# IuvenisSapiens/Qwen3-TTS-Rust

Hardware: AMD Instinct MI355X
Metric: audio-seconds generated per second (aggregate over GPUs) = concurrent real-time streams; RTF and first-chunk latency from the single-utterance leg (higher is better)
Workload: dtype i8

## Files before the change

### include/q3tts.h

```cpp
#ifndef Q3TTS_H
#define Q3TTS_H
#include <stdint.h>
#include <stddef.h>
#ifdef __cplusplus
extern "C" {
#endif

#define Q3TTS_OK 0
#define Q3TTS_ERR -1

const char* q3tts_last_error(void);
int q3tts_version(void);
int q3tts_device_count(void);

typedef struct q3tts_sampler_config {
    float temperature;
    int32_t top_k;
    float top_p;
    int32_t has_seed;
    uint64_t seed;
} q3tts_sampler_config;
void q3tts_sampler_config_default(q3tts_sampler_config* c);

typedef struct q3tts_gen_options {
// ... 236 lines not shown
int32_t q3tts_tokenizer_vocab_size(q3tts_tokenizer* t);
int64_t q3tts_text_nfc(const char* utf8, char* out, int64_t cap);

typedef struct q3tts_onnx q3tts_onnx;
int q3tts_onnx_open(const char* path, q3tts_onnx** out);
void q3tts_onnx_close(q3tts_onnx* m);
int q3tts_onnx_counts(q3tts_onnx* m, int32_t* n_nodes, int32_t* n_initializers, int32_t* n_inputs, int32_t* n_outputs);
int64_t q3tts_onnx_summary(q3tts_onnx* m, char* buf, int64_t cap);
int q3tts_onnx_node(q3tts_onnx* m, int32_t i, const char** op_type, const char** name, int32_t* n_in, int32_t* n_out, int32_t* n_attr);
const char* q3tts_onnx_node_input(q3tts_onnx* m, int32_t i, int32_t j);
const char* q3tts_onnx_node_output(q3tts_onnx* m, int32_t i, int32_t j);
int32_t q3tts_onnx_node_attr_ints(q3tts_onnx* m, int32_t i, const char* attr, int64_t* out, int32_t cap);
int32_t q3tts_onnx_node_attr_float(q3tts_onnx* m, int32_t i, const char* attr, float* out);
int q3tts_onnx_initializer(q3tts_onnx* m, int32_t i, const char** name, int32_t* dtype, int64_t* dims8, int32_t* ndims, const void** data,
                           int64_t* nbytes);
const char* q3tts_onnx_op_kernel(const char* op_type);
int q3tts_onnx_decoder_contract(q3tts_onnx* m, char* buf, int64_t cap);

typedef struct q3tts_onnx_session q3tts_onnx_session;
int q3tts_onnx_session_open(const char* path, int32_t device, q3tts_onnx_session** out);
void q3tts_onnx_session_close(q3tts_onnx_session* s);
int32_t q3tts_onnx_session_unsupported(q3tts_onnx_session* s, char* buf, int64_t cap);
int q3tts_onnx_session_set_input(q3tts_onnx_session* s, const char* name, int32_t dtype, const void* data, const int64_t* shape, int32_t rank);
int q3tts_onnx_session_run(q3tts_onnx_session* s);
int q3tts_onnx_session_output_info(q3tts_onnx_session* s, const char* name, int32_t* dtype, int32_t* rank, int64_t* shape8);
int q3tts_onnx_session_output(q3tts_onnx_session* s, const char* name, void* dst, int64_t cap_bytes);
int64_t q3tts_onnx_session_launches(q3tts_onnx_session* s);
int q3tts_onnx_op_executable(const char* op_type);
typedef struct q3tts_onnx_decoder q3tts_onnx_decoder;
int q3tts_onnx_decoder_open(const char* path, int32_t device, q3tts_onnx_decoder** out);
void q3tts_onnx_decoder_close(q3tts_onnx_decoder* d);
int q3tts_onnx_decoder_reset(q3tts_onnx_decoder* d);
int q3tts_onnx_decoder_decode(q3tts_onnx_decoder* d, const int64_t* codes, int32_t n_frames, int32_t is_final, float* pcm, int64_t cap, int64_t* n_out);
int q3tts_onnx_decoder_fetch(q3tts_onnx_decoder* d, float* pcm, int64_t cap, int64_t* n_out);

int q3tts_op_gemv_q8(const void* w_q8_0 , int32_t n, int32_t k, const int8_t* xq,
                     const uint16_t* xd, int32_t ntok, float* y , int32_t lpr);
int q3tts_op_gemv_kq(const void* const* raws, const int32_t* types, const int32_t* rows, int32_t nparts, int32_t k, const int8_t* xq, const uint16_t* xd,
                     int32_t ntok, float* y, int32_t lpr);
int q3tts_op_gateup_kq(const void* gate_raw, const void* up_raw, int32_t type, int32_t ff, int32_t k, const int8_t* xq, const uint16_t* xd, int32_t ntok,
                       int8_t* aq, uint16_t* ad);
int q3tts_op_gateup_q8(const void* w_q8_0, int32_t ff, int32_t k, const int8_t* xq, const uint16_t* xd, int32_t ntok, int8_t* aq,
                       uint16_t* ad);
int q3tts_op_matmul_float(const void* w , int32_t type, int32_t n, int32_t k, int32_t row0, int32_t nrows,
                          const float* x , int32_t ntok, float* y );
int q3tts_op_rmsnorm_quant(const float* x, const float* g, int32_t d, int32_t ntok, float eps, int8_t* xq, uint16_t* xd,
                           float* xn);
int q3tts_op_swiglu_quant(const float* gu, int32_t ff, int32_t ntok, int8_t* aq, uint16_t* ad);
int q3tts_op_argmax(const float* logits, int32_t n, int32_t start, int32_t end, int32_t mask_idx, int32_t* out);
int q3tts_op_sample(const float* logits, int32_t n, float temperature, int32_t top_k, float top_p, uint64_t seed, int32_t mask_idx,
                    int32_t n_draws, int32_t* out);
int q3tts_op_sample_rows(int32_t kernel, const float* logits, int32_t B, int32_t n, const float* temperature, const int32_t* top_k,
                         const float* top_p, const float* penalty, const uint64_t* seed, const int32_t* hist, const int32_t* hist_len,
                         int32_t hist_cap, int32_t n_draws, int32_t* out);
int q3tts_op_project(const float* x, const float* w , const float* b, int32_t n_in, int32_t n_out, float* y);
int q3tts_op_logprob_rows(const float* logits, int32_t B, int32_t n, int32_t stride, const int32_t* chosen, int32_t extra_idx,
                          float* out_chosen, float* out_extra);
int q3tts_op_score_rows(const float* tlogits, int32_t t_stride, const float* plogits, const int32_t* codes, int32_t F, float* out);
int q3tts_op_score_inputs(const float* hidden_proj, const float* const* tabs, const int64_t* tab_rows, int32_t dP, const int32_t* codes,
                          int32_t F, float* out);
int q3tts_op_kv_fork(uint16_t* k_cache, uint16_t* v_cache, int32_t n_pages, int32_t n_layer, int32_t n_kv, const int32_t* page_table,
                     int32_t n_seq, int32_t max_pages, int32_t src_seq, const int32_t* dst_seqs, int32_t n_dst, int32_t n_positions);
int q3tts_op_feedback_rows(const q3tts_assets* a, const int32_t* codes, int32_t n, const int32_t* trail_ids, int32_t n_trail, float* rows);
enum { Q3TTS_GEMM_AUTO = 0, Q3TTS_GEMM_SKINNY4 = 1, Q3TTS_GEMM_SKINNY8 = 2, Q3TTS_GEMM_SKINNY16 = 3,
       Q3TTS_GEMM_F32_1 = 4, Q3TTS_GEMM_F32_2 = 5,
       Q3TTS_GEMM_H1 = 6, Q3TTS_GEMM_H1_EPL = 7, Q3TTS_GEMM_H2 = 8, Q3TTS_GEMM_H2_EPL = 9,
       Q3TTS_GEMM_H3 = 10, Q3TTS_GEMM_H3_EPL = 11 };
enum { Q3TTS_EPI_NONE = 0, Q3TTS_EPI_GELU = 1, Q3TTS_EPI_RES_SCALE = 2 , Q3TTS_EPI_RES = 3 ,
       Q3TTS_EPI_SNAKE = 4  };
typedef struct q3tts_codec_gemm_desc {
    int32_t M, N, cin, taps, dil;
    const float* A; int64_t a_rows; int32_t lda, a_segT, a_skip;
    int32_t a_split, o_split;
    const float* W; const float* bias;
    int32_t epi; const float* res; int64_t res_floats; int32_t ldr, r_segT; int64_t r_skip;
    const float* scale; const float* snake_ea; const float* snake_ib;
    float* out; int64_t out_floats, out_off; int32_t ldo, o_segT; int64_t o_skip;
    int64_t ws_floats;
    int32_t form, ksplit, reducer;
    int32_t form_ran, ksplit_ran, reducer_ran;
} q3tts_codec_gemm_desc;
int q3tts_op_codec_gemm(q3tts_codec_gemm_desc* d);
int q3tts_codec_gemm_plan(q3tts_codec_gemm_desc* d);

enum { Q3TTS_CK_RVQ_SUM = 0, Q3TTS_CK_RMSNORM_ROWS = 1, Q3TTS_CK_LAYERNORM_ROWS = 2, Q3TTS_CK_ROPE_APPEND = 3, Q3TTS_CK_WINDOW_ATTN = 4,
       Q3TTS_CK_SWIGLU_ROWS = 5, Q3TTS_CK_DWCONV7 = 6, Q3TTS_CK_SNAKE = 7, Q3TTS_CK_SNAKE_SPLIT = 8, Q3TTS_CK_CONV_OUT_WAVE = 9,
       Q3TTS_CK_CONV_OUT_WIN = 10, Q3TTS_CK_HIST_LOAD = 11, Q3TTS_CK_HIST_SAVE = 12, Q3TTS_CK_HIST_ZERO = 13 };
typedef struct q3tts_codec_kernel_desc {
    int32_t kernel;
    int32_t G, T, C, H;
    int32_t n_heads, head_dim, window; float rope_base, eps, bias;
    const int64_t* meta;
    const int64_t* codes; int32_t n_q, cb_size;
    int32_t n_streams, stream;
    const float* in[3]; int64_t in_floats[3];
    const float* p0; const float* p1; int64_t p0_floats, p1_floats;
    float* out[3]; int64_t out_floats[3];
} q3tts_codec_kernel_desc;
int q3tts_op_codec_kernel(q3tts_codec_kernel_desc* d);

enum { Q3TTS_ATTN_AUTO = 0, Q3TTS_ATTN_UNFUSED = 1 , Q3TTS_ATTN_FUSED = 2 ,
       Q3TTS_ATTN_SHORT1 = 3, Q3TTS_ATTN_SHORT2 = 4 , Q3TTS_ATTN_GGML = 5  };
typedef struct q3tts_attention_desc {
    int32_t n_head, n_kv, n_layer, layer, ntok;
    const float* qkv; int32_t qkv_stride;
    const float* q_norm; const float* k_norm;
    float eps, rope_base; int32_t n_ctx; int32_t mrope_sec[4];
    const int32_t* seq; const int32_t* slot; const int32_t* pos; int32_t uniform_pos;
    const int32_t* page_table; int32_t n_seq, max_pages;
    uint16_t* k_cache; uint16_t* v_cache; int32_t n_pages;
    int32_t fused, fused_max_tok, same_seq, short_attn_min, hpw1_max, float_mode, ggml_mode;
    int32_t form;
    float* att; int8_t* aq; uint16_t* ad;
    int32_t form_ran;
} q3tts_attention_desc;
int q3tts_op_attention(q3tts_attention_desc* d);
int q3tts_op_attention_keyed(q3tts_attention_desc* d, const uint64_t* keys, int32_t key_stride, int32_t qkv_rows);
int q3tts_attention_plan(q3tts_attention_desc* d);

enum { Q3TTS_LOP_GEMV = 0, Q3TTS_LOP_GATEUP = 1, Q3TTS_LOP_NORM = 2, Q3TTS_LOP_NORM_GEMV = 3, Q3TTS_LOP_NORM_ARGMAX = 4, Q3TTS_LOP_NORM_GATEUP = 5,
       Q3TTS_LOP_F_GEMV = 6, Q3TTS_LOP_F_GATEUP = 7 };
enum { Q3TTS_LIN_AUTO = 0, Q3TTS_LIN_GEMV_Q8 = 1, Q3TTS_LIN_GEMM_Q8_TOK = 2, Q3TTS_LIN_GEMM_Q8_MFMA = 3, Q3TTS_LIN_GEMM_Q8_TILE1 = 4,
       Q3TTS_LIN_GEMV_KQ = 5, Q3TTS_LIN_GEMM_KQ_MFMA = 6, Q3TTS_LIN_GU_Q8_TILE1 = 7, Q3TTS_LIN_GU_Q8_MFMA = 8, Q3TTS_LIN_GU_KQ_MFMA = 9,
       Q3TTS_LIN_GU_UNFUSED = 10, Q3TTS_LIN_NORM = 11, Q3TTS_LIN_NORM_WG = 12, Q3TTS_LIN_GEMV_NORM = 13, Q3TTS_LIN_GEMV_NORM_ARGMAX = 14,
       Q3TTS_LIN_GU_SWIGLU_NORM = 15, Q3TTS_LIN_F_GEMV = 16, Q3TTS_LIN_F_MFMA16 = 17, Q3TTS_LIN_F_MFMA = 18, Q3TTS_LIN_F_GU_MFMA16 = 19,
       Q3TTS_LIN_F_GU_UNFUSED = 20 };
typedef struct q3tts_linear_desc {
    int32_t op, form;
    int32_t nw; const void* raw[3]; int32_t type[3]; int32_t rows[3]; int32_t kq_layout;
    int32_t K, row0, nrows, nrows_valid, ntok, ff;
    int32_t lpr, mt, ztiles;
    int32_t fused;
    const int8_t* xq; const uint16_t* xd; int32_t a_rows;
    const float* x; int64_t x_floats; int32_t x_off, x_stride;
    const float* h_in; int64_t h_floats; int32_t h_stride;
    const uint64_t* idx_keys; const int32_t* idx; int32_t idx_stride;
    const float* parts; int64_t parts_floats; int32_t nparts, parts_stride; int64_t parts_slab;
    const float* g; float eps;
    float* h_out; float* xn_out;
    int8_t* xq_out; uint16_t* xd_out;
    uint64_t* keys; int64_t n_keys; int32_t key_stride; const int32_t* mask_per_tok; int32_t idx_add;
    float* out; int64_t out_floats, out_off; int32_t out_stride;
    int8_t* aq; uint16_t* ad;
    int32_t form_ran, lpr_ran, mt_ran, z_ran;
} q3tts_linear_desc;
int q3tts_op_linear(q3tts_linear_desc* d);
int q3tts_linear_plan(q3tts_linear_desc* d);
uint64_t q3tts_argmax_key(float v, int32_t idx);

enum { Q3TTS_SEL_SAMPLE = 0, Q3TTS_SEL_SAMPLE_PRED = 1, Q3TTS_SEL_ARGMAX = 2, Q3TTS_SEL_ARGMAX_KEYS = 3 };
#define Q3TTS_SELECT_SENTINEL 0xA5C3F00D5A3C0FF1ull
typedef struct q3tts_select_desc {
    int32_t kernel;
    int32_t B, n, stride, row_off;
    const float* logits;
    const float* temperature; const int32_t* top_k; const float* top_p;
    const int32_t* mask_idx;
    const uint64_t* seed;
    const uint32_t* draw0;
    int32_t n_draws;
    const float* penalty; const int32_t* hist; const int32_t* hist_len; int32_t hist_cap; const int32_t* cur_code;
    int32_t out_stride;
    int32_t start, end, add;
    int32_t* tokens;
    uint64_t* out_raw;
    uint32_t* draws_out;
// ... 8 lines not shown
```

### qwen3-tts-rust_amd/csrc/capi_ops.cpp

```cpp
#include "../../include/q3tts.h"
#include "transformer.h"
#include "host_logic.h"
#include "kdev.h"
#include "codec.h"

using namespace q3;
#define Q3_API_BEGIN try {
#define Q3_API_END(failval) } catch (const std::exception& ex) { set_last_error(ex.what()); return failval; } catch (...) { set_last_error("unknown error"); return failval; }
static void require_gpu() {
    int n = 0;
    if (hipGetDeviceCount(&n) != hipSuccess || n <= 0) throw Error("no HIP device available: the HIP path is the only compute path (no CPU fallback)");
}

static int attention_op_plan(const q3tts_attention_desc& d) {
    AttnPlanIn a;
    a.ntok = d.ntok; a.fused = d.fused != 0; a.fused_max_tok = d.fused_max_tok; a.same_seq = d.same_seq != 0; a.short_attn_min = d.short_attn_min;
    a.n_head = d.n_head; a.n_kv = d.n_kv; a.hpw1_max = d.hpw1_max > 0 ? d.hpw1_max : short_attn_hpw1_max();
    a.float_mode = d.float_mode != 0; a.ggml_mode = d.ggml_mode != 0;
    return plan_attention(a);
}

static void attention_op_check(const q3tts_attention_desc& d, int form) {
    Q3_CHECK(form >= ATTN_UNFUSED && form <= ATTN_GGML, "unknown attention form");
    Q3_CHECK(d.n_head >= 1 && d.n_kv >= 1 && d.n_head % d.n_kv == 0, "n_head must be a multiple of n_kv");
// ... 718 lines not shown
        Q3_CHECK(d.hist && d.hist_len && d.hist_cap >= 1, "a penalty needs a history");
        for (int b = 0; b < B; b++) Q3_CHECK(d.hist_len[b] >= 0 && d.hist_len[b] <= d.hist_cap, "hist_len out of range");
    }
    const float guard = 3e38f;
    std::vector<float> hl((size_t)d.row_off + (size_t)B * d.stride, guard);
    for (int b = 0; b < B; b++) std::copy(d.logits + (size_t)b * n, d.logits + (size_t)(b + 1) * n, hl.begin() + d.row_off + (size_t)b * d.stride);
    DevBuf<float> dl(hl.size()); dl.upload(hl.data(), hl.size());
    const float* rows = dl.p + d.row_off;
    DevBuf<int32_t> dm;
    if (d.mask_idx) { dm.alloc(B); dm.upload(d.mask_idx, B); }
    const size_t slots = (size_t)B * d.out_stride;
    std::vector<q3_u64> raw((size_t)nl * slots);
    if (d.kernel == Q3TTS_SEL_ARGMAX) {
        const int32_t s32 = (int32_t)(uint32_t)(Q3TTS_SELECT_SENTINEL & 0xFFFFFFFFull);
        std::vector<int32_t> ho(slots, s32);
        DevBuf<int32_t> dout(slots); dout.upload(ho.data(), slots);
        launch_argmax(0, rows, d.stride, d.start, d.end, dm.p, dout.p, d.out_stride, d.add, B);
        Q3_LAUNCH_CHECK();
        Q3_HIP(hipDeviceSynchronize());
        dout.download(ho.data(), slots);
        for (size_t i = 0; i < slots; i++) raw[i] = (q3_u64)(uint32_t)ho[i];
        std::copy(raw.begin(), raw.end(), (q3_u64*)d.out_raw);
        for (int b = 0; b < B; b++) d.tokens[b] = ho[(size_t)b * d.out_stride];
        return Q3TTS_OK;
    }
    std::fill(raw.begin(), raw.end(), (q3_u64)Q3TTS_SELECT_SENTINEL);
    DevBuf<q3_u64> dout(raw.size()); dout.upload(raw.data(), raw.size());
    if (d.kernel == Q3TTS_SEL_ARGMAX_KEYS) {
        launch_argmax_keys(0, rows, d.stride, n, dm.p, dout.p, d.out_stride, B);
        Q3_LAUNCH_CHECK();
        Q3_HIP(hipDeviceSynchronize());
        dout.download((q3_u64*)d.out_raw, raw.size());
        for (int b = 0; b < B; b++) d.tokens[b] = key_code(d.out_raw[(size_t)b * d.out_stride]);
        return Q3TTS_OK;
    }
    DevBuf<float> dt(B), dp_(B), dpen; DevBuf<int32_t> dk(B), dh, dlen; DevBuf<uint32_t> dkey((size_t)8 * B), ddraw(B); DevBuf<q3_u64> dcur;
    dt.upload(d.temperature, B); dp_.upload(d.top_p, B); dk.upload(d.top_k, B);
    std::vector<uint32_t> keys((size_t)8 * B), draw(B, 0u);
    for (int b = 0; b < B; b++) { StdRng rng(d.seed[b]); std::copy(rng.key(), rng.key() + 8, keys.begin() + (size_t)b * 8); if (d.draw0) draw[b] = d.draw0[b]; }
    dkey.upload(keys.data(), keys.size()); ddraw.upload(draw.data(), B);
    SampleArgs a{rows, d.stride, n, dt.p, dk.p, dp_.p, dm.p, dkey.p, ddraw.p, dout.p, d.out_stride};
    if (d.penalty) {
        const size_t hs = (size_t)d.hist_cap * 16;
        std::vector<int32_t> hh((size_t)B * hs, 0);
        for (int b = 0; b < B; b++) for (int f = 0; f < d.hist_cap; f++) hh[(size_t)b * hs + (size_t)f * 16] = d.hist[(size_t)b * d.hist_cap + f];
        dh.alloc(hh.size()); dh.upload(hh.data(), hh.size()); dlen.alloc(B); dlen.upload(d.hist_len, B); dpen.alloc(B); dpen.upload(d.penalty, B);
        a.penalty = dpen.p; a.hist = dh.p; a.hist_stride = (int)hs; a.hist_len = dlen.p;
        if (d.cur_code) {
            std::vector<q3_u64> cur((size_t)16 * B, pack_key(0.0f, 0));
            for (int b = 0; b < B; b++) cur[(size_t)b * 16] = pack_key(0.0f, d.cur_code[b]);
            dcur.alloc(cur.size()); dcur.upload(cur.data(), cur.size());
            a.cur_key = dcur.p; a.cur_stride = 16;
        }
    }
    for (int i = 0; i < nl; i++) {
        a.out_key = dout.p + (size_t)i * slots;
        if (d.kernel == Q3TTS_SEL_SAMPLE) launch_sample(0, a, B);
        else launch_sample_pred(0, a, B);
        Q3_LAUNCH_CHECK();
    }
    Q3_HIP(hipDeviceSynchronize());
    dout.download((q3_u64*)d.out_raw, raw.size());
    ddraw.download(d.draws_out, B);
    for (int i = 0; i < nl; i++) for (int b = 0; b < B; b++) d.tokens[(size_t)i * B + b] = key_code(d.out_raw[(size_t)i * slots + (size_t)b * d.out_stride]);
    return Q3TTS_OK;
    Q3_API_END(Q3TTS_ERR)
}

int q3tts_op_codec_gemm(q3tts_codec_gemm_desc* d) {
    Q3_API_BEGIN
    require_gpu();
    codec_gemm_run(d);
    return Q3TTS_OK;
    Q3_API_END(Q3TTS_ERR)
}

int q3tts_codec_gemm_plan(q3tts_codec_gemm_desc* d) {
    Q3_API_BEGIN
    codec_gemm_plan_only(d);
    return Q3TTS_OK;
    Q3_API_END(Q3TTS_ERR)
}

int q3tts_op_codec_kernel(q3tts_codec_kernel_desc* d) {
    Q3_API_BEGIN
    require_gpu();
    codec_kernel_run(d);
    return Q3TTS_OK;
    Q3_API_END(Q3TTS_ERR)
}

int q3tts_op_project(const float* x, const float* w, const float* b, int32_t n_in, int32_t n_out, float* y) {
    Q3_API_BEGIN
    require_gpu();
    std::vector<float> wt((size_t)n_in * n_out);
    for (int o = 0; o < n_out; o++) for (int i = 0; i < n_in; i++) wt[(size_t)i * n_out + o] = w[(size_t)o * n_in + i];
    DevBuf<float> dx(n_in), dw(wt.size()), db(n_out), dy(n_out);
    dx.upload(x, n_in); dw.upload(wt.data(), wt.size()); db.upload(b, n_out);
    launch_project(0, dx.p, n_in, dw.p, db.p, n_in, n_out, dy.p, n_out, 1);
    Q3_HIP(hipDeviceSynchronize());
    dy.download(y, n_out);
    return Q3TTS_OK;
    Q3_API_END(Q3TTS_ERR)
}

int q3tts_mel_frames(int32_t n) { const int plen = n + 768; return (plen > 1024 ? plen - 1024 : 0) / 256 + 1; }

}

#include "onnx_reader.h"
#include "onnx_exec.h"
struct q3tts_onnx { std::unique_ptr<OnnxModel> m; std::string text; };
extern "C" {
int q3tts_onnx_open(const char* path, q3tts_onnx** out) {
    Q3_API_BEGIN
    Q3_CHECK(path && out, "null argument");
    auto* h = new q3tts_onnx();
    try { h->m.reset(new OnnxModel(path)); } catch (...) { delete h; throw; }
    *out = h;
    return Q3TTS_OK;
    Q3_API_END(Q3TTS_ERR)
}
void q3tts_onnx_close(q3tts_onnx* m) { delete m; }
int q3tts_onnx_counts(q3tts_onnx* m, int32_t* n_nodes, int32_t* n_init, int32_t* n_in, int32_t* n_out) {
    if (!m) return Q3TTS_ERR;
    if (n_nodes) *n_nodes = (int32_t)m->m->nodes.size();
    if (n_init) *n_init = (int32_t)m->m->initializers.size();
    if (n_in) *n_in = (int32_t)m->m->inputs.size();
    if (n_out) *n_out = (int32_t)m->m->outputs.size();
    return Q3TTS_OK;
}
int64_t q3tts_onnx_summary(q3tts_onnx* m, char* buf, int64_t cap) {
    if (!m) return -1;
    m->text = m->m->summary();
    if (buf && cap > 0) { const size_t n = std::min((size_t)cap - 1, m->text.size()); std::memcpy(buf, m->text.data(), n); buf[n] = 0; }
    return (int64_t)m->text.size() + 1;
}
int q3tts_onnx_node(q3tts_onnx* m, int32_t i, const char** op_type, const char** name, int32_t* n_in, int32_t* n_out, int32_t* n_attr) {
    Q3_API_BEGIN
    Q3_CHECK(m && i >= 0 && i < (int)m->m->nodes.size(), "node index out of range");
    const OnnxNode& n = m->m->nodes[i];
    if (op_type) *op_type = n.op_type.c_str();
    if (name) *name = n.name.c_str();
    if (n_in) *n_in = (int32_t)n.inputs.size();
    if (n_out) *n_out = (int32_t)n.outputs.size();
    if (n_attr) *n_attr = (int32_t)n.attrs.size();
    return Q3TTS_OK;
    Q3_API_END(Q3TTS_ERR)
}
const char* q3tts_onnx_node_input(q3tts_onnx* m, int32_t i, int32_t j) {
    return (m && i >= 0 && i < (int)m->m->nodes.size() && j >= 0 && j < (int)m->m->nodes[i].inputs.size()) ? m->m->nodes[i].inputs[j].c_str() : nullptr;
}
const char* q3tts_onnx_node_output(q3tts_onnx* m, int32_t i, int32_t j) {
    return (m && i >= 0 && i < (int)m->m->nodes.size() && j >= 0 && j < (int)m->m->nodes[i].outputs.size()) ? m->m->nodes[i].outputs[j].c_str() : nullptr;
}
int32_t q3tts_onnx_node_attr_ints(q3tts_onnx* m, int32_t i, const char* attr, int64_t* out, int32_t cap) {
    if (!m || i < 0 || i >= (int)m->m->nodes.size() || !attr) return -1;
    const OnnxAttr* a = m->m->nodes[i].attr(attr);
    if (!a) return -1;
    if (a->type == 2 || (a->ints.empty() && a->type == 0)) { if (out && cap > 0) out[0] = a->i; return 1; }
    for (int k = 0; k < (int)a->ints.size() && k < cap; k++) out[k] = a->ints[k];
    return (int32_t)a->ints.size();
}
int32_t q3tts_onnx_node_attr_float(q3tts_onnx* m, int32_t i, const char* attr, float* out) {
    if (!m || i < 0 || i >= (int)m->m->nodes.size() || !attr || !out) return -1;
    const OnnxAttr* a = m->m->nodes[i].attr(attr);
// ... 164 lines not shown
```

### qwen3-tts-rust_amd/csrc/codec.h

```cpp
#pragma once
#include "q3_common.h"
#include <memory>
#include <string>
#include <vector>

struct q3tts_codec_gemm_desc;
struct q3tts_codec_kernel_desc;

namespace q3 {

struct CodecStateEntry { std::string name; int64_t offset; int rows, cols; };

class CodecDecoder {
public:
    std::vector<CodecStateEntry> state_layout() const;
    size_t state_floats() const;
    void state_export(int stream, float* out, size_t n_floats) const;
    void state_import(int stream, const float* in, size_t n_floats);
    CodecDecoder(const std::string& gguf_path, int n_streams, int max_frames_per_call, int n_lanes = 1, int max_group = 1);
    int max_group() const;
    int n_lanes() const;
    ~CodecDecoder();
    int samples_per_frame() const;
    void reset(int stream);
    void reset_async(hipStream_t st, int stream);
    int decode(hipStream_t st, int stream, const int64_t* codes, int n_frames, bool is_last, float* pcm);
    int decode_async(hipStream_t st, int stream, const int64_t* codes, int n_frames, bool is_last, float* pcm_pinned, int lane = 0);
    int decode_group_async(hipStream_t st, int G, const int* streams, const int64_t* codes, int n_frames, float* const* pcm_pinned, int lane = 0);
    double flops_per_frame() const;
private:
    struct Impl;
    std::unique_ptr<Impl> impl_;
};

void codec_gemm_run(q3tts_codec_gemm_desc* d);
void codec_gemm_plan_only(q3tts_codec_gemm_desc* d);
void codec_kernel_run(q3tts_codec_kernel_desc* d);

}
```

### qwen3-tts-rust_amd/csrc/codec.hip

```cpp
#include "codec.h"
#include "../../include/q3tts.h"
#include "gguf.h"
#include <cmath>
#include <cstdlib>
#include <map>

namespace q3 {

typedef float f32x16 __attribute__((ext_vector_type(16)));

enum { EPI_NONE = 0, EPI_GELU = 1, EPI_RES_SCALE = 2, EPI_RES = 3, EPI_SNAKE = 4 };

struct GemmArgs {
    const float* A; int lda;
    int cin, dil;
    const float* W;
    const float* wscale;
    const float* bias;
    float* out; int ldo;
    int M, N, K;
    int epi; const float* res; int ldr; const float* scale;
    const float *snake_ea, *snake_ib;
    float* ws;
    int a_segT, a_skip; int o_segT; long long o_skip; int r_segT; long long r_skip;
    int a_split, o_split;
    int xcd_swizzle;
};
#define SEG_NONE 0x3fffffff

__device__ __forceinline__ int seg_of(int row, int segT) { return segT == SEG_NONE ? 0 : row / segT; }
__device__ __forceinline__ size_t out_off(const GemmArgs& g, int row, int col) { return (size_t)row * g.ldo + (size_t)seg_of(row, g.o_segT) * g.o_skip + col; }
typedef _Float16 h4v_ __attribute__((ext_vector_type(4)));
__device__ __forceinline__ float4 load_a4(const GemmArgs& g, size_t row, int ci) {
    if (!g.a_split) return *reinterpret_cast<const float4*>(g.A + row * g.lda + ci);
    const _Float16* base = reinterpret_cast<const _Float16*>(g.A + row * g.lda);
    const h4v_ hi = *reinterpret_cast<const h4v_*>(base + ci), lo = *reinterpret_cast<const h4v_*>(base + g.cin + ci);
    return make_float4((float)hi[0] + (float)lo[0], (float)hi[1] + (float)lo[1], (float)hi[2] + (float)lo[2], (float)hi[3] + (float)lo[3]);
}
__device__ __forceinline__ float4 load_a4_split_raw(const GemmArgs& g, size_t row, int ci) {
    const _Float16* base = reinterpret_cast<const _Float16*>(g.A + row * g.lda);
    const float2 hi = *reinterpret_cast<const float2*>(base + ci), lo = *reinterpret_cast<const float2*>(base + g.cin + ci);
    return make_float4(hi.x, hi.y, lo.x, lo.y);
}
__device__ __forceinline__ void gemm_store(const GemmArgs& g, int row, int col, float v) {
    const size_t o = out_off(g, row, 0);
    if (!g.o_split) { g.out[o + col] = v; return; }
    _Float16* base = reinterpret_cast<_Float16*>(g.out + o);
    const _Float16 hi = (_Float16)v;
    base[col] = hi; base[g.N + col] = (_Float16)(v - (float)hi);
}

__device__ __forceinline__ float snake_sin(float x) {
    const float n = rintf(x * 0.63661977236758134f);
    float r = fmaf(n, -1.57079637050628662f, x);
    r = fmaf(n, 4.37113900018624283e-8f, r);
    const int q = (int)n;
    const float r2 = r * r;
    const float sp = fmaf(fmaf(fmaf(-1.9515295891e-4f, r2, 8.3321608736e-3f), r2, -1.6666654611e-1f), r2 * r, r);
    const float cp = fmaf(fmaf(fmaf(2.443315711809948e-5f, r2, -1.388731625493765e-3f), r2, 4.166664568298827e-2f), r2 * r2, fmaf(-0.5f, r2, 1.0f));
    const float v = (q & 1) ? cp : sp;
    return (q & 2) ? -v : v;
}
__device__ __forceinline__ float gemm_epilogue(const GemmArgs& g, float v, int row, int col) {
    if (g.bias) v += g.bias[col];
    if (g.epi == EPI_GELU) v = 0.5f * v * (1.0f + erff(v * 0.70710678118654752f));
    else if (g.epi == EPI_RES_SCALE) v = g.res[(size_t)row * g.ldr + (size_t)seg_of(row, g.r_segT) * g.r_skip + col] + g.scale[col] * v;
    else if (g.epi == EPI_RES) v = g.res[(size_t)row * g.ldr + (size_t)seg_of(row, g.r_segT) * g.r_skip + col] + v;
    else if (g.epi == EPI_SNAKE) { const float sn = snake_sin(v * g.snake_ea[col]); v = v + g.snake_ib[col] * (sn * sn); }
    return v;
}

typedef _Float16 h4e_ __attribute__((ext_vector_type(4)));
__device__ __forceinline__ void gemm_epilogue_store4(const GemmArgs& g, float4 t, int row, int col) {
    float v[4] = {t.x, t.y, t.z, t.w};
    if (g.bias) { const float4 b = *reinterpret_cast<const float4*>(g.bias + col); v[0] += b.x; v[1] += b.y; v[2] += b.z; v[3] += b.w; }
    if (g.epi == EPI_GELU) {
#pragma unroll
        for (int c = 0; c < 4; c++) v[c] = 0.5f * v[c] * (1.0f + erff(v[c] * 0.70710678118654752f));
    } else if (g.epi == EPI_RES_SCALE || g.epi == EPI_RES) {
        const float4 rs = *reinterpret_cast<const float4*>(g.res + (size_t)row * g.ldr + (size_t)seg_of(row, g.r_segT) * g.r_skip + col);
        if (g.epi == EPI_RES_SCALE) {
            const float4 sc = *reinterpret_cast<const float4*>(g.scale + col);
            v[0] = rs.x + sc.x * v[0]; v[1] = rs.y + sc.y * v[1]; v[2] = rs.z + sc.z * v[2]; v[3] = rs.w + sc.w * v[3];
        } else { v[0] = rs.x + v[0]; v[1] = rs.y + v[1]; v[2] = rs.z + v[2]; v[3] = rs.w + v[3]; }
    } else if (g.epi == EPI_SNAKE) {
        const float4 ea = *reinterpret_cast<const float4*>(g.snake_ea + col), ib = *reinterpret_cast<const float4*>(g.snake_ib + col);
        const float eav[4] = {ea.x, ea.y, ea.z, ea.w}, ibv[4] = {ib.x, ib.y, ib.z, ib.w};
#pragma unroll
        for (int c = 0; c < 4; c++) { const float sn = snake_sin(v[c] * eav[c]); v[c] = v[c] + ibv[c] * (sn * sn); }
    }
    const size_t o = out_off(g, row, 0);
    if (!g.o_split) *reinterpret_cast<float4*>(g.out + o + col) = make_float4(v[0], v[1], v[2], v[3]);
    else {
        _Float16* base = reinterpret_cast<_Float16*>(g.out + o);
        h4e_ hi, lo;
#pragma unroll
        for (int c = 0; c < 4; c++) { hi[c] = (_Float16)v[c]; lo[c] = (_Float16)(v[c] - (float)hi[c]); }
        *reinterpret_cast<h4e_*>(base + col) = hi;
        *reinterpret_cast<h4e_*>(base + g.N + col) = lo;
    }
}
static bool epilogue4_ok(const GemmArgs& g) {
    auto a16 = [](const void* p) { return (reinterpret_cast<uintptr_t>(p) & 15) == 0; };
    return g.N % 4 == 0 && g.ldo % 4 == 0 && g.o_skip % 4 == 0 && a16(g.out) && (!g.bias || a16(g.bias)) &&
           (!(g.epi == EPI_RES || g.epi == EPI_RES_SCALE) || (g.ldr % 4 == 0 && g.r_skip % 4 == 0 && a16(g.res))) &&
           (g.epi != EPI_RES_SCALE || a16(g.scale)) && (g.epi != EPI_SNAKE || (a16(g.snake_ea) && a16(g.snake_ib)));
}

template <int WM>
__global__ void __launch_bounds__(256) k_conv_gemm(GemmArgs g) {
    constexpr int WN = 4 / WM, BM = 32 * WM, BN = 32 * WN, BK = 16;
    constexpr int NA = BM * 4 / 256 > 0 ? BM * 4 / 256 : 1, NB = BN * 4 / 256 > 0 ? BN * 4 / 256 : 1;
    __shared__ float As[BK][BM];
    __shared__ float Bs[BK][BN];
    const int tid = threadIdx.x, lane = tid & 63, wave = tid >> 6;
    const int wm = wave / WN, wn = wave % WN;
    const int m0 = blockIdx.y * BM, n0 = blockIdx.x * BN;
    const int ksplit = gridDim.z, kper = g.K / ksplit, kbeg = blockIdx.z * kper, kend = kbeg + kper;
    f32x16 acc;
#pragma unroll
    for (int i = 0; i < 16; i++) acc[i] = 0.0f;
    float4 ra[NA], rb[NB];
    int arow[NA];
#pragma unroll
    for (int i = 0; i < NA; i++) { const int mm = m0 + (tid + i * 256) % BM; arow[i] = mm + seg_of(mm, g.a_segT) * g.a_skip; }
    auto fetch = [&](int k0) {
        const int j = k0 / g.cin, ci0 = k0 % g.cin;
#pragma unroll
        for (int i = 0; i < NA; i++) {
            const int e = tid + i * 256, r = e % BM, qd = e / BM;
            ra[i] = make_float4(0.f, 0.f, 0.f, 0.f);
            if (e < BM * 4 && m0 + r < g.M) ra[i] = load_a4(g, (size_t)(arow[i] + j * g.dil), ci0 + 4 * qd);
        }
#pragma unroll
        for (int i = 0; i < NB; i++) {
            const int e = tid + i * 256, r = e % BN, qd = e / BN;
            rb[i] = make_float4(0.f, 0.f, 0.f, 0.f);
            if (e < BN * 4 && n0 + r < g.N) rb[i] = *reinterpret_cast<const float4*>(g.W + (size_t)(n0 + r) * g.K + k0 + 4 * qd);
        }
    };
    auto stash = [&]() {
#pragma unroll
        for (int i = 0; i < NA; i++) {
            const int e = tid + i * 256, r = e % BM, qd = e / BM;
            if (e < BM * 4) { As[4 * qd + 0][r] = ra[i].x; As[4 * qd + 1][r] = ra[i].y; As[4 * qd + 2][r] = ra[i].z; As[4 * qd + 3][r] = ra[i].w; }
        }
#pragma unroll
        for (int i = 0; i < NB; i++) {
            const int e = tid + i * 256, r = e % BN, qd = e / BN;
            if (e < BN * 4) { Bs[4 * qd + 0][r] = rb[i].x; Bs[4 * qd + 1][r] = rb[i].y; Bs[4 * qd + 2][r] = rb[i].z; Bs[4 * qd + 3][r] = rb[i].w; }
        }
    };
    fetch(kbeg);
    for (int k0 = kbeg; k0 < kend; k0 += BK) {
        stash();
        __syncthreads();
        if (k0 + BK < kend) fetch(k0 + BK);
#pragma unroll
        for (int kk = 0; kk < BK; kk += 2) {
            const float a = As[kk + (lane >> 5)][wm * 32 + (lane & 31)];
            const float b = Bs[kk + (lane >> 5)][wn * 32 + (lane & 31)];
            acc = __builtin_amdgcn_mfma_f32_32x32x2f32(a, b, acc, 0, 0, 0);
        }
        __syncthreads();
    }
    const int col = n0 + wn * 32 + (lane & 31);
    if (col < g.N) {
#pragma unroll
        for (int r = 0; r < 16; r++) {
            const int row = m0 + wm * 32 + (r & 3) + 8 * (r >> 2) + 4 * (lane >> 5);
            if (row < g.M) {
                if (ksplit > 1) g.ws[((size_t)blockIdx.z * g.M + row) * g.N + col] = acc[r];
                else gemm_store(g, row, col, gemm_epilogue(g, acc[r], row, col));
            }
        }
    }
}
typedef _Float16 h8v __attribute__((ext_vector_type(8)));
typedef _Float16 h4v __attribute__((ext_vector_type(4)));
template <int MR, int EPL, bool SPLIT>
__global__ void __launch_bounds__(256) k_conv_gemm_h(GemmArgs g, const _Float16* __restrict__ Wh, const _Float16* __restrict__ Wl) {
    constexpr int BM = 64 * MR, BN = 64, BK = 32, LD = 40;
    constexpr int NA = BM * 8 / 256;
    constexpr int CLD = BN + 4;
    struct Stage { _Float16 Ah[BM][LD], Al[BM][LD], Bh[BN][LD], Bl[BN][LD]; };
    union Shared { Stage s; float Ct[EPL ? BM : 1][CLD]; };
    __shared__ __attribute__((aligned(16))) Shared sh;
    auto& Ah = sh.s.Ah; auto& Al = sh.s.Al; auto& Bh = sh.s.Bh; auto& Bl = sh.s.Bl;
    const int tid = threadIdx.x, lane = tid & 63, wave = tid >> 6;
// ... 202 lines not shown
#pragma unroll
                for (int u = 0; u < NT; u++) {
                    bh[u] = *reinterpret_cast<const h8v*>(&Bh[u * 32 + (lane & 31)][ko]);
                    bl[u] = *reinterpret_cast<const h8v*>(&Bl[u * 32 + (lane & 31)][ko]);
                }
#pragma unroll
                for (int t = 0; t < MR; t++) {
                    const int ar = (wave * MR + t) * 32 + (lane & 31);
                    const h8v ah = *reinterpret_cast<const h8v*>(&Ah[ar][ko]);
                    const h8v al = *reinterpret_cast<const h8v*>(&Al[ar][ko]);
#pragma unroll
                    for (int u = 0; u < NT; u++) {
                        acc[t][u] = __builtin_amdgcn_mfma_f32_32x32x16_f16(al, bh[u], acc[t][u], 0, 0, 0);
                        acc[t][u] = __builtin_amdgcn_mfma_f32_32x32x16_f16(ah, bl[u], acc[t][u], 0, 0, 0);
                        acc[t][u] = __builtin_amdgcn_mfma_f32_32x32x16_f16(ah, bh[u], acc[t][u], 0, 0, 0);
                    }
                    __builtin_amdgcn_sched_barrier(0);
                }
            }
        }
    };
    auto lds_barrier = [] { asm volatile("s_waitcnt lgkmcnt(0)\n\ts_barrier" ::: "memory"); };
    float wsc[NT];
#pragma unroll
    for (int u = 0; u < NT; u++) wsc[u] = g.wscale[n0 + u * 32 + (lane & 31)];
    Regs st[PF];
#pragma unroll
    for (int j = 0; j < PF; j++)
        if (kbeg + j * BK < kend) fetch(st[j], kbeg + j * BK);
    int k0 = kbeg;
    for (; k0 + 2 * PF * BK <= kend; k0 += PF * BK) {
#pragma unroll
        for (int j = 0; j < PF; j++) {
            stash(st[j]);
            lds_barrier();
            fetch(st[j], k0 + (j + PF) * BK);
            multiply();
            lds_barrier();
        }
    }
    for (; k0 < kend; k0 += PF * BK) {
#pragma unroll
        for (int j = 0; j < PF; j++) {
            if (k0 + j * BK < kend) {
                stash(st[j]);
                lds_barrier();
                if (k0 + (j + PF) * BK < kend) fetch(st[j], k0 + (j + PF) * BK);
                multiply();
                lds_barrier();
            }
        }
    }
#pragma unroll
    for (int u = 0; u < NT; u++)
#pragma unroll
        for (int t = 0; t < MR; t++)
#pragma unroll
            for (int r = 0; r < 16; r++) acc[t][u][r] *= wsc[u];
    __syncthreads();
    auto epilogue_rows = [&](const f32x16 (&a)[NT], int row0) {
#pragma unroll
        for (int r = 0; r < 16; r++) {
            const int row = row0 + (r & 3) + 8 * (r >> 2) + 4 * (lane >> 5);
            if (row < g.M) {
#pragma unroll
                for (int u = 0; u < NT; u++) {
                    const int col = n0 + u * 32 + (lane & 31);
                    if (col < g.N) {
                        if (ksplit > 1) g.ws[((size_t)blockIdx.z * g.M + row) * g.N + col] = a[u][r];
                        else gemm_store(g, row, col, gemm_epilogue(g, a[u][r], row, col));
                    }
                }
            }
        }
    };
    if constexpr (EPL != 0 && MR == 1) {
        auto& Ct = sh.Ct;
#pragma unroll
        for (int u = 0; u < NT; u++)
#pragma unroll
            for (int r = 0; r < 16; r++) Ct[wave * 32 + (r & 3) + 8 * (r >> 2) + 4 * (lane >> 5)][u * 32 + (lane & 31)] = acc[0][u][r];
        __syncthreads();
        constexpr int C4 = BN / 4;
        for (int e = tid; e < BM * C4; e += 256) {
            const int rl = e / C4, col = n0 + (e % C4) * 4, row = m0 + rl;
            if (row >= g.M) continue;
            const float4 t4 = *reinterpret_cast<const float4*>(&Ct[rl][(e % C4) * 4]);
            if (ksplit > 1) *reinterpret_cast<float4*>(g.ws + ((size_t)blockIdx.z * g.M + row) * g.N + col) = t4;
            else gemm_epilogue_store4(g, t4, row, col);
        }
    } else {
        epilogue_rows(acc[0], m0 + wave * MR * 32);
        if constexpr (MR > 1) epilogue_rows(acc[1], m0 + (wave * MR + 1) * 32);
    }
    static_assert(MR <= 2, "one epilogue call per row tile");
}
__global__ void __launch_bounds__(256) k_splitk_reduce4(GemmArgs g, int ksplit) {
    const size_t i = ((size_t)blockIdx.x * 256 + threadIdx.x) * 4, mn = (size_t)g.M * g.N;
    if (i >= mn) return;
    const int row = (int)(i / g.N), col = (int)(i % g.N);
    float4 v = *reinterpret_cast<const float4*>(g.ws + i);
    for (int s = 1; s < ksplit; s++) {
        const float4 w = *reinterpret_cast<const float4*>(g.ws + (size_t)s * mn + i);
        v.x += w.x; v.y += w.y; v.z += w.z; v.w += w.w;
    }
    gemm_epilogue_store4(g, v, row, col);
}
__global__ void __launch_bounds__(256) k_splitk_reduce(GemmArgs g, int ksplit) {
    const size_t i = (size_t)blockIdx.x * 256 + threadIdx.x;
    if (i >= (size_t)g.M * g.N) return;
    const int row = (int)(i / g.N), col = (int)(i % g.N);
    float v = g.ws[i];
    for (int s = 1; s < ksplit; s++) v += g.ws[(size_t)s * g.M * g.N + i];
    gemm_store(g, row, col, gemm_epilogue(g, v, row, col));
}

template <int MT>
__global__ void __launch_bounds__(512) k_skinny_gemm(GemmArgs g) {
    constexpr int KT = 512;
    __shared__ __attribute__((aligned(16))) float As[MT][KT];
    const int tid = threadIdx.x, lane = tid & 63, wave = tid >> 6;
    const int n = blockIdx.x * 8 + wave;
    const int nn = n < g.N ? n : g.N - 1;
    float acc[MT];
#pragma unroll
    for (int m = 0; m < MT; m++) acc[m] = 0.0f;
    for (int k0 = 0; k0 < g.K; k0 += KT) {
        const int kt = (g.K - k0) < KT ? (g.K - k0) : KT;
        float4 w4[2];
#pragma unroll
        for (int i = 0; i < 2; i++) {
            const int kk = 4 * (lane + 64 * i);
            w4[i] = (kk < kt) ? *reinterpret_cast<const float4*>(g.W + (size_t)nn * g.K + k0 + kk) : make_float4(0.f, 0.f, 0.f, 0.f);
        }
        __syncthreads();
        for (int e = tid; e < MT * (KT / 4); e += 512) {
            const int m = e / (KT / 4), kk = 4 * (e % (KT / 4));
            float4 v = make_float4(0.f, 0.f, 0.f, 0.f);
            if (m < g.M && kk < kt) {
                const int kg = k0 + kk, j = kg / g.cin, ci = kg % g.cin;
                v = load_a4(g, (size_t)(m + seg_of(m, g.a_segT) * g.a_skip + j * g.dil), ci);
            }
            *reinterpret_cast<float4*>(&As[m][kk]) = v;
        }
        __syncthreads();
#pragma unroll
        for (int i = 0; i < 2; i++) {
            const int kk = 4 * (lane + 64 * i);
#pragma unroll
            for (int m = 0; m < MT; m++) {
                const float4 a = *reinterpret_cast<const float4*>(&As[m][kk]);
                acc[m] += w4[i].x * a.x + w4[i].y * a.y + w4[i].z * a.z + w4[i].w * a.w;
            }
        }
    }
    float mine = 0.0f;
#pragma unroll
    for (int m = 0; m < MT; m++) {
        float v = acc[m];
        for (int o = 32; o >= 1; o >>= 1) v += __shfl_xor(v, o);
        if (lane == m) mine = v;
    }
    if (lane < MT && lane < g.M && n < g.N) gemm_store(g, lane, n, gemm_epilogue(g, mine, lane, n));
}
static const bool g_codec_f32 = [] { const char* e = std::getenv("Q3_CODEC_F32"); return e && e[0] == '1'; }();
struct GemmPlan { int form, ks, red; };
static GemmPlan plan_gemm(const GemmArgs& g, size_t ws_floats, bool has_split_w) {
    if (g.M <= 16) return GemmPlan{g.M <= 4 ? Q3TTS_GEMM_SKINNY4 : g.M <= 8 ? Q3TTS_GEMM_SKINNY8 : Q3TTS_GEMM_SKINNY16, 1, -1};
    const bool small = g.M <= 32;
    const int tiles = small ? ((g.N + 127) / 128) * ((g.M + 31) / 32) : ((g.N + 63) / 64) * ((g.M + 63) / 64);
    int ksplit = 1;
    while (tiles * ksplit < 256 && ksplit < 16 && (g.K / (ksplit * 2)) % 16 == 0 && g.K / (ksplit * 2) >= 128 &&
           (size_t)(ksplit * 2) * g.M * g.N <= ws_floats) ksplit *= 2;
    const bool ws_a16 = (reinterpret_cast<uintptr_t>(g.ws) & 15) == 0;
    static const int h3_min_wgs = [] { const char* e = std::getenv("Q3_CODEC_H3_MIN_WGS"); return e ? atoi(e) : 128; }();
    static const int h3_max_n = [] { const char* e = std::getenv("Q3_CODEC_H3_MAXN"); return e ? atoi(e) : 1 << 30; }();
    static const int epl_on = [] { const char* e = std::getenv("Q3_CODEC_H3_EPL"); return e ? atoi(e) : 1; }();
    static const int h3_wgs = [] { const char* e = std::getenv("Q3_CODEC_H3_WGS"); return e ? atoi(e) : 0; }();
    static const int h3_min_tiles = [] { const char* e = std::getenv("Q3_CODEC_H3_MIN_TILES"); return e ? atoi(e) : 96; }();
    if (!small && has_split_w && !g_codec_f32 && g.cin % 32 == 0 && h3_min_wgs > 0 && g.N % 96 == 0 && g.N <= h3_max_n) {
        const int tiles3 = (g.N / 96) * ((g.M + 127) / 128);
        const bool vec_ok = epl_on && epilogue4_ok(g) && ws_a16;
        int ks = 1;
        if (vec_ok && h3_wgs > 0 && tiles3 >= h3_min_tiles && tiles3 < h3_wgs) {
            static const int cand[] = {2, 3, 4, 6, 7, 8, 12, 14, 16};
            for (int c : cand) {
                if (g.K % c != 0 || (g.K / c) % 32 != 0 || g.K / c < 256 || (size_t)c * g.M * g.N > ws_floats) continue;
                ks = c;
                if (tiles3 * c >= h3_wgs) break;
            }
        }
        if (tiles3 * ks >= h3_min_wgs) return GemmPlan{vec_ok ? Q3TTS_GEMM_H3_EPL : Q3TTS_GEMM_H3, ks, ks > 1 ? 1 : -1};
    }
    if (!small && has_split_w && !g_codec_f32 && g.cin % 32 == 0) {
        static const int big_m = [] { const char* e = std::getenv("Q3_CODEC_BM128"); return e ? atoi(e) : 1024; }();
        const bool tall = g.M >= big_m && g.N >= 512 && ((g.N + 63) / 64) * ((g.M + 127) / 128) >= 160;
        const int t2 = tall ? ((g.N + 63) / 64) * ((g.M + 127) / 128) : tiles;
        static const int wg_target = [] { const char* e = std::getenv("Q3_CODEC_WGS"); return e ? atoi(e) : 256; }();
        int ks = 1;
        while (t2 * ks < wg_target && ks < 16 && (g.K / (ks * 2)) % 32 == 0 && g.K / (ks * 2) >= 128 && (size_t)(ks * 2) * g.M * g.N <= ws_floats) ks *= 2;
        static const int epl4 = [] { const char* e = std::getenv("Q3_CODEC_EPL4"); return e ? atoi(e) : 1; }();
        const bool vec_ok = epl4 && epilogue4_ok(g) && ws_a16;
        const int form = tall ? (vec_ok ? Q3TTS_GEMM_H2_EPL : Q3TTS_GEMM_H2) : (vec_ok ? Q3TTS_GEMM_H1_EPL : Q3TTS_GEMM_H1);
        return GemmPlan{form, ks, ks > 1 ? (vec_ok ? 1 : 0) : -1};
    }
    return GemmPlan{small ? Q3TTS_GEMM_F32_1 : Q3TTS_GEMM_F32_2, ksplit, ksplit > 1 ? 0 : -1};
}
static const char* gemm_plan_error(const GemmArgs& g, const GemmPlan& p, size_t ws_floats, bool has_split_w) {
    const int f = p.form;
    if (f < Q3TTS_GEMM_SKINNY4 || f > Q3TTS_GEMM_H3_EPL) return "unknown GEMM form";
    if (g.M < 1 || g.N < 1 || g.cin < 4 || g.K % g.cin != 0 || g.dil < 1) return "bad GEMM shape";
    if (g.cin % 4 != 0 || g.lda % 4 != 0 || g.lda < g.cin) return "A rows need cin % 4 == 0 and lda % 4 == 0, lda >= cin";
    if (p.ks < 1 || g.K % p.ks != 0) return "ksplit must divide K";
    const bool skinny = f <= Q3TTS_GEMM_SKINNY16, f32 = f == Q3TTS_GEMM_F32_1 || f == Q3TTS_GEMM_F32_2, h3 = f >= Q3TTS_GEMM_H3;
    const bool epl = f == Q3TTS_GEMM_H1_EPL || f == Q3TTS_GEMM_H2_EPL || f == Q3TTS_GEMM_H3_EPL;
    const bool ws_a16 = (reinterpret_cast<uintptr_t>(g.ws) & 15) == 0;
    if (skinny) {
        if (g.M > (f == Q3TTS_GEMM_SKINNY4 ? 4 : f == Q3TTS_GEMM_SKINNY8 ? 8 : 16)) return "skinny form: M exceeds its row count";
        if (p.ks != 1) return "skinny form: no split-K";
        return nullptr;
    }
    if (f32 && (g.cin % 16 != 0 || (g.K / p.ks) % 16 != 0)) return "f32 form: cin and K / ksplit must be multiples of 16";
    if (!f32) {
        if (!has_split_w || !g.wscale) return "split-f16 form without split weights";
        if (g.cin % 32 != 0 || (g.K / p.ks) % 32 != 0) return "split-f16 form: cin and K / ksplit must be multiples of 32";
        if (h3 && g.N % 96 != 0) return "h3 form: N must be a multiple of 96";
        if (epl && !(epilogue4_ok(g) && ws_a16)) return "16-byte epilogue form: pointers / strides not 16-byte aligned or N % 4 != 0";
    }
    if (p.ks > 1) {
        if (p.ks > 64) return "ksplit too large";
        if ((size_t)p.ks * g.M * g.N > ws_floats) return "split-K workspace too small";
        if (p.red != 0 && p.red != 1) return "split-K needs a reducer (0 or 1)";
        if (p.red == 1 && !(epilogue4_ok(g) && ws_a16)) return "k_splitk_reduce4: pointers / strides not 16-byte aligned or N % 4 != 0";
    } else if (p.red != -1) return "a reducer without split-K";
    return nullptr;
}
static void launch_gemm(hipStream_t st, const GemmArgs& g, const GemmPlan& p, const _Float16* wh, const _Float16* wl) {
    const dim3 b256(256);
    const unsigned ks = (unsigned)p.ks;
#define Q3_H(MRV, EPLV, GRID) do { if (g.a_split) hipLaunchKernelGGL((k_conv_gemm_h<MRV, EPLV, true>), GRID, b256, 0, st, g, wh, wl); \
                                   else hipLaunchKernelGGL((k_conv_gemm_h<MRV, EPLV, false>), GRID, b256, 0, st, g, wh, wl); } while (0)
#define Q3_H3(EPLV, PFV) do { if (g.a_split) hipLaunchKernelGGL((k_conv_gemm_h3<1, 3, 32, EPLV, PFV, true>), grid3, b256, 0, st, g, wh, wl); \
                              else hipLaunchKernelGGL((k_conv_gemm_h3<1, 3, 32, EPLV, PFV, false>), grid3, b256, 0, st, g, wh, wl); } while (0)
    const dim3 grid_sk((g.N + 7) / 8), grid_t((g.N + 63) / 64, (g.M + 127) / 128, ks), grid_s((g.N + 63) / 64, (g.M + 63) / 64, ks);
    const dim3 grid3(g.N / 96, (g.M + 127) / 128, ks);
    switch (p.form) {
    case Q3TTS_GEMM_SKINNY4: hipLaunchKernelGGL((k_skinny_gemm<4>), grid_sk, dim3(512), 0, st, g); break;
    case Q3TTS_GEMM_SKINNY8: hipLaunchKernelGGL((k_skinny_gemm<8>), grid_sk, dim3(512), 0, st, g); break;
    case Q3TTS_GEMM_SKINNY16: hipLaunchKernelGGL((k_skinny_gemm<16>), grid_sk, dim3(512), 0, st, g); break;
    case Q3TTS_GEMM_F32_1: hipLaunchKernelGGL((k_conv_gemm<1>), dim3((g.N + 127) / 128, (g.M + 31) / 32, ks), b256, 0, st, g); break;
    case Q3TTS_GEMM_F32_2: hipLaunchKernelGGL((k_conv_gemm<2>), dim3((g.N + 63) / 64, (g.M + 63) / 64, ks), b256, 0, st, g); break;
    case Q3TTS_GEMM_H1: Q3_H(1, 0, grid_s); break;
    case Q3TTS_GEMM_H1_EPL: Q3_H(1, 1, grid_s); break;
    case Q3TTS_GEMM_H2: Q3_H(2, 0, grid_t); break;
    case Q3TTS_GEMM_H2_EPL: Q3_H(2, 1, grid_t); break;
    case Q3TTS_GEMM_H3: Q3_H3(0, 1); break;
    case Q3TTS_GEMM_H3_EPL: Q3_H3(1, 1); break;
    default: throw Error("unknown GEMM form");
    }
#undef Q3_H
#undef Q3_H3
    if (p.ks > 1) {
        const size_t n = (size_t)g.M * g.N;
        if (p.red == 1) hipLaunchKernelGGL(k_splitk_reduce4, dim3((unsigned)((n / 4 + 255) / 256)), b256, 0, st, g, p.ks);
        else hipLaunchKernelGGL(k_splitk_reduce, dim3((unsigned)((n + 255) / 256)), b256, 0, st, g, p.ks);
    }
}
static int xcd_swizzle_on() { static const int on = [] { const char* e = std::getenv("Q3_CODEC_XCD"); return e ? atoi(e) : 1; }(); return on; }
static void gemm(hipStream_t st, GemmArgs g, float* ws, size_t ws_floats, const _Float16* wh = nullptr, const _Float16* wl = nullptr) {
    g.ws = ws;
    g.xcd_swizzle = xcd_swizzle_on();
    launch_gemm(st, g, plan_gemm(g, ws_floats, wh != nullptr), wh, wl);
}

struct RowMap { int segT, skip, off; };
__device__ __forceinline__ size_t map_row(const RowMap& m, int r) { return (size_t)r + (size_t)(m.segT == SEG_NONE ? 0 : r / m.segT) * m.skip + m.off; }
static RowMap plain_map() { return RowMap{SEG_NONE, 0, 0}; }

__global__ void k_rvq_sum(const int64_t* __restrict__ codes, const float* const* __restrict__ cb, int n_q, int cb_size, int cb_dim,
                          float* __restrict__ out, int ldo, RowMap om) {
    const int t = blockIdx.y, d = blockIdx.x * 256 + threadIdx.x;
    if (d >= cb_dim) return;
    float acc = 0.0f;
    for (int q = 0; q < n_q; q++) {
        long long c = codes[(size_t)t * n_q + q];
        c = c < 0 ? 0 : (c >= cb_size ? cb_size - 1 : c);
        acc += cb[q][(size_t)c * cb_dim + d];
    }
    out[map_row(om, t) * ldo + d] = acc;
}
__global__ void __launch_bounds__(256) k_rmsnorm_rows(const float* __restrict__ x, int ldx, const float* __restrict__ g, int C, float eps,
                                                      float* __restrict__ y, int ldy) {
    __shared__ float red[4];
    const int t = blockIdx.x;
    float s = 0.0f;
    for (int c = threadIdx.x; c < C; c += 256) { const float v = x[(size_t)t * ldx + c]; s += v * v; }
// ... 28 lines not shown
    const int r = blockIdx.y, e = blockIdx.x * 256 + threadIdx.x, half = hd / 2;
    if (e >= H / 2) return;
    const int head = e / half, i = e % half;
    const long long p = meta[2 * G + r / T0] + (r % T0);
    const float c = cs[(size_t)p * half + i], s = sn[(size_t)p * half + i];
    const size_t o = map_row(om, r) * H;
    float* row = qkv + (size_t)r * ld;
    {
        float* v = row + head * hd;
        const float a = v[i], b = v[i + half];
        v[i] = a * c - b * s; v[i + half] = b * c + a * s;
    }
    {
        float* v = row + H + head * hd;
        const float a = v[i], b = v[i + half];
        const float x = a * c - b * s, y = b * c + a * s;
        v[i] = x; v[i + half] = y;
        kext[o + head * hd + i] = x; kext[o + head * hd + i + half] = y;
    }
    vext[o + e] = row[2 * H + e];
    vext[o + e + H / 2] = row[2 * H + e + H / 2];
}
__global__ void __launch_bounds__(64) k_codec_attn(const float* __restrict__ qkv, int ld, int H, int hd, const float* __restrict__ kext,
                                                   const float* __restrict__ vext, const int64_t* __restrict__ meta, int G, int T0, int W,
                                                   float* __restrict__ out, int ldo) {
    __shared__ float p_s[128];
    __shared__ float q_s[128];
    const int head = blockIdx.x, r = blockIdx.y, lane = threadIdx.x;
    const int g = r / T0, t = r % T0;
    const int kvl = (int)meta[G + g];
    const size_t seg = (size_t)g * (W - 1 + T0);
    const int j1 = W - 1 + t, jv = W - 1 - kvl, j0 = t > jv ? t : jv, nk = j1 - j0 + 1;
    for (int d = lane; d < hd; d += 64) q_s[d] = qkv[(size_t)r * ld + head * hd + d];
    __syncthreads();
    const float scale = 1.0f / sqrtf((float)hd);
    float mx = -INFINITY;
    for (int jj = lane; jj < nk; jj += 64) {
        const float* kr = kext + (seg + j0 + jj) * H + head * hd;
        float a = 0.0f;
        if ((hd & 3) == 0) {
            for (int d = 0; d < hd; d += 4) {
                const float4 kk = *reinterpret_cast<const float4*>(kr + d);
                a += q_s[d] * kk.x; a += q_s[d + 1] * kk.y; a += q_s[d + 2] * kk.z; a += q_s[d + 3] * kk.w;
            }
        } else for (int d = 0; d < hd; d++) a += q_s[d] * kr[d];
        a *= scale;
        p_s[jj] = a;
        mx = fmaxf(mx, a);
    }
    for (int o = 32; o >= 1; o >>= 1) mx = fmaxf(mx, __shfl_xor(mx, o));
    float den = 0.0f;
    for (int jj = lane; jj < nk; jj += 64) { const float e = expf(p_s[jj] - mx); p_s[jj] = e; den += e; }
    for (int o = 32; o >= 1; o >>= 1) den += __shfl_xor(den, o);
    __syncthreads();
    for (int d = lane; d < hd; d += 64) {
        float a = 0.0f;
        for (int jj = 0; jj < nk; jj++) a += p_s[jj] * vext[(seg + j0 + jj) * H + head * hd + d];
        out[(size_t)r * ldo + head * hd + d] = a / den;
    }
}
__global__ void k_swiglu_rows(const float* __restrict__ gu, int ff, float* __restrict__ out) {
    const int t = blockIdx.y, c = blockIdx.x * 256 + threadIdx.x;
    if (c >= ff) return;
    const float g = gu[(size_t)t * 2 * ff + c], u = gu[(size_t)t * 2 * ff + ff + c];
    out[(size_t)t * ff + c] = (g / (1.0f + expf(-g))) * u;
}
__global__ void k_dwconv7(const float* __restrict__ in_ext, int C, const float* __restrict__ w, const float* __restrict__ b,
                          float* __restrict__ out, RowMap im) {
    const int t = blockIdx.y, c = blockIdx.x * 256 + threadIdx.x;
    if (c >= C) return;
    const size_t r0 = map_row(im, t);
    float a = b[c];
#pragma unroll
    for (int j = 0; j < 7; j++) a += w[c * 7 + j] * in_ext[(r0 + j) * C + c];
    out[(size_t)t * C + c] = a;
}
__global__ void k_snake(const float* __restrict__ src, float* __restrict__ dst, int C, const float* __restrict__ ea,
                        const float* __restrict__ inv_eb, size_t n4, RowMap dm, int split) {
    const size_t i = (size_t)blockIdx.x * 256 + threadIdx.x;
    if (i >= n4) return;
    const int c4 = C >> 2, c = (int)(i % c4) * 4, r = (int)(i / c4);
    const float4 v = reinterpret_cast<const float4*>(src)[i];
    const float4 a = *reinterpret_cast<const float4*>(ea + c), b = *reinterpret_cast<const float4*>(inv_eb + c);
    const float s0 = snake_sin(v.x * a.x), s1 = snake_sin(v.y * a.y), s2 = snake_sin(v.z * a.z), s3 = snake_sin(v.w * a.w);
    const float4 y = make_float4(v.x + b.x * (s0 * s0), v.y + b.y * (s1 * s1), v.z + b.z * (s2 * s2), v.w + b.w * (s3 * s3));
    float* drow = dst + map_row(dm, r) * C;
    if (!split) { *reinterpret_cast<float4*>(drow + c) = y; return; }
    _Float16* row = reinterpret_cast<_Float16*>(drow);
    h4v_ hi, lo;
    hi[0] = (_Float16)y.x; hi[1] = (_Float16)y.y; hi[2] = (_Float16)y.z; hi[3] = (_Float16)y.w;
    lo[0] = (_Float16)(y.x - (float)hi[0]); lo[1] = (_Float16)(y.y - (float)hi[1]); lo[2] = (_Float16)(y.z - (float)hi[2]); lo[3] = (_Float16)(y.w - (float)hi[3]);
    *reinterpret_cast<h4v_*>(row + c) = hi; *reinterpret_cast<h4v_*>(row + C + c) = lo;
}
__global__ void k_copy_rows(const float* __restrict__ src, float* __restrict__ dst, size_t n, int C, RowMap dm) {
    const size_t i = (size_t)blockIdx.x * 256 + threadIdx.x;
    if (i >= n) return;
    const int c = (int)(i % C), r = (int)(i / C);
    dst[map_row(dm, r) * C + c] = src[i];
}
struct HistDesc { float* work; float* hist; int H, C, T, pad; };
struct HistTable { HistDesc d[48]; int n; };
__global__ void k_hist_all(HistTable tab, const int64_t* __restrict__ meta, int save) {
    const HistDesc e = tab.d[blockIdx.z];
    const int g = blockIdx.y;
    const size_t n = (size_t)e.H * e.C, i = ((size_t)blockIdx.x * 256 + threadIdx.x) * 4;
    if (i >= n) return;
    float* w = e.work + (size_t)g * (e.H + e.T) * e.C;
    float* h = e.hist + (size_t)meta[g] * n;
    if (save) *reinterpret_cast<float4*>(h + i) = *reinterpret_cast<const float4*>(w + (size_t)e.T * e.C + i);
    else *reinterpret_cast<float4*>(w + i) = *reinterpret_cast<const float4*>(h + i);
}
__global__ void k_hist_zero(HistTable tab, int stream) {
    const HistDesc e = tab.d[blockIdx.z];
    const size_t n = (size_t)e.H * e.C, i = (size_t)blockIdx.x * 256 + threadIdx.x;
    if (i < n) e.hist[(size_t)stream * n + i] = 0.0f;
}
__global__ void __launch_bounds__(256) k_conv_out_wave(const float* __restrict__ in_ext, int C, const float* __restrict__ w, float bias,
                                                       float* __restrict__ pcm, int n, RowMap im) {
    const int t = blockIdx.x * 4 + (threadIdx.x >> 6), lane = threadIdx.x & 63;
    if (t >= n) return;
    const float* row = in_ext + map_row(im, t) * C;
    float a = 0.0f;
    for (int i = lane; i < 7 * C / 4; i += 64) {
        const float4 x = *reinterpret_cast<const float4*>(row + 4 * i), ww = *reinterpret_cast<const float4*>(w + 4 * i);
        a += ww.x * x.x + ww.y * x.y + ww.z * x.z + ww.w * x.w;
    }
    for (int o = 32; o >= 1; o >>= 1) a += __shfl_xor(a, o);
    a += bias;
    if (lane == 0) pcm[t] = a < -1.0f ? -1.0f : (a > 1.0f ? 1.0f : a);
}
template <int C>
__global__ void __launch_bounds__(256) k_conv_out_win(const float* __restrict__ in_ext, const float* __restrict__ w, float bias, float* __restrict__ pcm, int n, RowMap im) {
    constexpr int TB = 128, ROWS = TB + 6, SPAN4 = 7 * C / 4, NW = (SPAN4 + 63) / 64;
    __shared__ __attribute__((aligned(16))) float xs[ROWS * C];
    const int t0 = blockIdx.x * TB, tid = threadIdx.x, lane = tid & 63, wave = tid >> 6;
    const float* src = in_ext + map_row(im, t0) * C;
    for (int e = tid; e < ROWS * C / 4; e += 256) *reinterpret_cast<float4*>(xs + 4 * e) = *reinterpret_cast<const float4*>(src + 4 * e);
    float4 wv[NW];
#pragma unroll
    for (int k = 0; k < NW; k++) { const int i = lane + 64 * k; wv[k] = i < SPAN4 ? *reinterpret_cast<const float4*>(w + 4 * i) : make_float4(0.f, 0.f, 0.f, 0.f); }
    __syncthreads();
    for (int j = 0; j < TB / 4; j++) {
        const int tl = wave * (TB / 4) + j;
        float a = 0.0f;
#pragma unroll
        for (int k = 0; k < NW; k++) {
            const int i = lane + 64 * k;
            if (i < SPAN4) {
                const float4 x = *reinterpret_cast<const float4*>(xs + tl * C + 4 * i);
                a += wv[k].x * x.x + wv[k].y * x.y + wv[k].z * x.z + wv[k].w * x.w;
            }
        }
        for (int o = 32; o >= 1; o >>= 1) a += __shfl_xor(a, o);
        a += bias;
        if (lane == 0 && t0 + tl < n) pcm[t0 + tl] = a < -1.0f ? -1.0f : (a > 1.0f ? 1.0f : a);
    }
}
static void launch_rvq_sum(hipStream_t st, const int64_t* codes, const float* const* cb, int n_q, int cb_size, int cb_dim, int R, float* out, RowMap om) {
    hipLaunchKernelGGL(k_rvq_sum, dim3((cb_dim + 255) / 256, R), dim3(256), 0, st, codes, cb, n_q, cb_size, cb_dim, out, cb_dim, om);
}
static void launch_rmsnorm(hipStream_t st, const float* x, const float* g, int C, float eps, float* y, int R) {
    hipLaunchKernelGGL(k_rmsnorm_rows, dim3(R), dim3(256), 0, st, x, C, g, C, eps, y, C);
}
static void launch_layernorm(hipStream_t st, const float* x, const float* w, const float* b, int C, float eps, float* y, int R) {
    hipLaunchKernelGGL(k_layernorm_rows, dim3(R), dim3(256), 0, st, x, C, w, b, C, eps, y, C);
}
static void launch_rope_append(hipStream_t st, float* qkv, int H, int hd, const float* cs, const float* sn, const int64_t* meta, int G, int T0,
                               float* kext, float* vext, RowMap om) {
    hipLaunchKernelGGL(k_codec_rope_append, dim3((H / 2 + 255) / 256, G * T0), dim3(256), 0, st, qkv, 3 * H, H, hd, cs, sn, meta, G, T0, kext, vext, om);
}
static void launch_window_attn(hipStream_t st, const float* qkv, int n_heads, int H, int hd, const float* kext, const float* vext, const int64_t* meta,
                               int G, int T0, int W, float* out) {
    hipLaunchKernelGGL(k_codec_attn, dim3(n_heads, G * T0), dim3(64), 0, st, qkv, 3 * H, H, hd, kext, vext, meta, G, T0, W, out, H);
}
static void launch_swiglu(hipStream_t st, const float* gu, int ff, float* out, int R) {
    hipLaunchKernelGGL(k_swiglu_rows, dim3((ff + 255) / 256, R), dim3(256), 0, st, gu, ff, out);
}
static void launch_dwconv7(hipStream_t st, const float* in_ext, int C, const float* w, const float* b, float* out, int R, RowMap im) {
    hipLaunchKernelGGL(k_dwconv7, dim3((C + 255) / 256, R), dim3(256), 0, st, in_ext, C, w, b, out, im);
}
static void launch_snake(hipStream_t st, const float* src, float* dst, int C, const float* ea, const float* inv_eb, int rows, RowMap dm, bool split) {
    const size_t n = (size_t)rows * (C / 4);
    hipLaunchKernelGGL(k_snake, dim3((unsigned)((n + 255) / 256)), dim3(256), 0, st, src, dst, C, ea, inv_eb, n, dm, split ? 1 : 0);
}
static bool conv_out_win_ok(int C, int T) { return C == 96 && T % 128 == 0; }
static void launch_conv_out(hipStream_t st, const float* in_ext, int C, const float* w, float bias, float* pcm, int G, int T, RowMap im, bool win) {
    if (win) hipLaunchKernelGGL((k_conv_out_win<96>), dim3(G * T / 128), dim3(256), 0, st, in_ext, w, bias, pcm, G * T, im);
    else hipLaunchKernelGGL(k_conv_out_wave, dim3((G * T + 3) / 4), dim3(256), 0, st, in_ext, C, w, bias, pcm, G * T, im);
}
static void launch_hist_all(hipStream_t st, const HistTable& tab, int G, const int64_t* meta, bool save) {
    size_t mx = 0;
    for (int i = 0; i < tab.n; i++) mx = std::max(mx, (size_t)tab.d[i].H * tab.d[i].C);
    hipLaunchKernelGGL(k_hist_all, dim3((unsigned)((mx / 4 + 255) / 256), G, tab.n), dim3(256), 0, st, tab, meta, save ? 1 : 0);
}
static void launch_hist_zero(hipStream_t st, const HistTable& tab, int stream) {
    size_t mx = 0;
    for (int i = 0; i < tab.n; i++) mx = std::max(mx, (size_t)tab.d[i].H * tab.d[i].C);
    hipLaunchKernelGGL(k_hist_zero, dim3((unsigned)((mx + 255) / 256), 1, tab.n), dim3(256), 0, st, tab, stream);
}
static void rope_tables(int hd, float base, int n_pos, std::vector<float>& c, std::vector<float>& s) {
    const int half = hd / 2;
    c.resize((size_t)n_pos * half); s.resize((size_t)n_pos * half);
    for (int i = 0; i < half; i++) {
        const double f = std::pow((double)base, -(double)i / half);
        for (int p = 0; p < n_pos; p++) { const double ang = (double)p * f; c[(size_t)p * half + i] = (float)std::cos(ang); s[(size_t)p * half + i] = (float)std::sin(ang); }
    }
}
static bool positions_ok(long long seen, int T0) { return seen >= 0 && T0 >= 0 && seen + T0 <= (long long)Q3TTS_CODEC_MAX_FRAMES; }

static void split_weights(const float* w, int N, int K, _Float16* wh, _Float16* wl, float* wscale) {
    for (int n = 0; n < N; n++) {
        const float* r = w + (size_t)n * K;
        float mx = 0.0f;
        for (int k = 0; k < K; k++) mx = std::max(mx, std::fabs(r[k]));
        int e = 0, s = 0;
        if (mx > 0.0f && std::isfinite(mx)) { std::frexp(mx, &e); s = std::min(14 - e, 126); }
        wscale[n] = std::ldexp(1.0f, -s);
        const float up = std::ldexp(1.0f, s);
        for (int k = 0; k < K; k++) {
            const float x = r[k] * up;
            const _Float16 h = (_Float16)x;
            wh[(size_t)n * K + k] = h; wl[(size_t)n * K + k] = (_Float16)(x - (float)h);
        }
    }
}
struct ConvW { DevBuf<float> w, b, wsc; DevBuf<_Float16> wh, wl; int N = 0, K = 0, cin = 0, taps = 1, dil = 1; };
struct Snake { DevBuf<float> ea, inv_eb; int C = 0; };
struct Ext { DevBuf<float> hist; int H = 0, C = 0, Tmax = 0, id = -1; };

struct CodecDecoder::Impl {
    int n_q, cb_size, cb_dim, hidden, n_layers, n_heads, head_dim, ffn, window, n_up, dec_dim, n_dec;
    int up_ratios[4], dec_rates[8];
    float rope_base, eps;
    int n_streams, max_frames;
    std::vector<DevBuf<float>> codebooks; DevBuf<const float*> d_cb_ptrs;
    ConvW pre_conv;
    struct TfL { DevBuf<float> attn_norm, ffn_norm, ls_attn, ls_ffn; ConvW wqkv, wo, wgu, wdown; };
    std::vector<TfL> tf; DevBuf<float> tf_norm, rope_c, rope_s;
    struct Up { ConvW ct, pw1, pw2; DevBuf<float> dw_w, dw_b, ln_w, ln_b, gamma; };
    std::vector<Up> up;
    ConvW conv_in;
    struct RU { Snake s1, s2; ConvW c1, c2; };
    struct Blk { Snake snake; ConvW ct; RU ru[3]; int cin, cout, rate; };
    std::vector<Blk> blk;
    Snake snake_out; DevBuf<float> conv_out_w; float conv_out_b = 0;
    Ext z_ext, convin_ext, out_ext; std::vector<Ext> dw_ext, ct_ext, k_ext, v_ext; std::vector<std::vector<Ext>> ru_ext;
    std::vector<Ext*> all_ext;
    bool presplit = false;
    std::vector<int> kv_len; std::vector<long long> n_seen;
    int gmax = 1;
    struct Scratch {
        DevBuf<float> h, xn, qkv, att, gu, act, t1, t2, pcm, splitk_ws; DevBuf<int64_t> d_in;
        std::vector<DevBuf<float>> work;
        int64_t* h_in = nullptr; int ring_idx = 0;
    };
    std::vector<Scratch> lanes; Scratch* S = nullptr; int ring = 256;
    size_t in_slot() const { return (size_t)gmax * max_frames * n_q + 3 * (size_t)gmax; }
    double flops_frame = 0;

    static std::vector<float> tensor(const Gguf& g, const std::string& name) {
        const GgufTensor& t = g.need(name);
        Q3_CHECK(t.type == Q3_T_F32, "codec tensor not F32: " + name);
        const float* p = reinterpret_cast<const float*>(t.data);
        return std::vector<float>(p, p + t.nbytes / 4);
    }
    static void up_f(DevBuf<float>& d, const std::vector<float>& v) { d.alloc(v.size()); d.upload(v.data(), v.size()); }
    static void split_w(ConvW& c, const std::vector<float>& r, int N) {
        const int K = (int)(r.size() / N);
        std::vector<_Float16> h(r.size()), l(r.size());
        std::vector<float> sc(N);
        split_weights(r.data(), N, K, h.data(), l.data(), sc.data());
        c.wh.alloc(h.size()); c.wh.upload(h.data(), h.size());
        c.wl.alloc(l.size()); c.wl.upload(l.data(), l.size());
        up_f(c.wsc, sc);
    }
    void make_conv(ConvW& c, const Gguf& g, const std::string& wn, const std::string& bn, int cout, int cin, int k, int dil) {
        auto w = tensor(g, wn);
        Q3_CHECK((int64_t)w.size() == (int64_t)cout * cin * k && cin % 16 == 0, "conv shape " + wn);
        std::vector<float> r((size_t)cout * cin * k);
        for (int co = 0; co < cout; co++) for (int ci = 0; ci < cin; ci++) for (int j = 0; j < k; j++)
            r[((size_t)co * k + j) * cin + ci] = w[((size_t)co * cin + ci) * k + j];
        up_f(c.w, r); split_w(c, r, cout);
        if (!bn.empty()) up_f(c.b, tensor(g, bn));
        c.N = cout; c.K = cin * k; c.cin = cin; c.taps = k; c.dil = dil;
    }
    void make_linear(ConvW& c, const std::vector<float>& w, int N, int K) { up_f(c.w, w); split_w(c, w, N); c.N = N; c.K = K; c.cin = K; c.taps = 1; c.dil = 1; }
    void make_convt(ConvW& c, const Gguf& g, const std::string& wn, const std::string& bn, int cin, int cout, int k, int s) {
        auto w = tensor(g, wn);
        auto b = tensor(g, bn);
        Q3_CHECK((int64_t)w.size() == (int64_t)cin * cout * k && (k == 2 * s || k == s) && cin % 16 == 0, "convT shape " + wn);
        const int taps = k / s;
        std::vector<float> r((size_t)s * cout * taps * cin), br((size_t)s * cout);
        for (int rr = 0; rr < s; rr++) for (int co = 0; co < cout; co++) {
            br[(size_t)rr * cout + co] = b[co];
            for (int ci = 0; ci < cin; ci++) {
                if (taps == 2) {
                    r[((size_t)(rr * cout + co) * 2 + 0) * cin + ci] = w[((size_t)ci * cout + co) * k + rr + s];
                    r[((size_t)(rr * cout + co) * 2 + 1) * cin + ci] = w[((size_t)ci * cout + co) * k + rr];
                } else r[(size_t)(rr * cout + co) * cin + ci] = w[((size_t)ci * cout + co) * k + rr];
            }
        }
        up_f(c.w, r); split_w(c, r, s * cout); up_f(c.b, br);
        c.N = s * cout; c.K = taps * cin; c.cin = cin; c.taps = taps; c.dil = 1;
    }
    void make_snake(Snake& s, const Gguf& g, const std::string& an, const std::string& bn, int C) {
        auto a = tensor(g, an), b = tensor(g, bn);
        std::vector<float> ea(C), ib(C);
        for (int i = 0; i < C; i++) { ea[i] = expf(a[i]); ib[i] = 1.0f / (expf(b[i]) + 1e-9f); }
        up_f(s.ea, ea); up_f(s.inv_eb, ib); s.C = C;
    }
    void make_ext(Ext& e, int H, int C, int Tmax) {
        e.H = H; e.C = C; e.Tmax = Tmax; e.id = (int)all_ext.size();
        e.hist.alloc((size_t)n_streams * H * C); e.hist.zero();
        all_ext.push_back(&e);
    }
    struct Loc { float* p; int segT; long long skip_rows; };
    Loc plain(float* p) { return Loc{p, SEG_NONE, 0}; }
    float* work(const Ext& e) { return S->work[e.id].p; }
    Loc ext_base(const Ext& e, int T) { return Loc{work(e), T, e.H}; }
    Loc ext_cur(const Ext& e, int T) { return Loc{work(e) + (size_t)e.H * e.C, T, e.H}; }
    RowMap cur_map(const Ext& e, int T) { return RowMap{T, e.H, e.H}; }
    RowMap base_map(const Ext& e, int T) { return RowMap{T, e.H, 0}; }
    void run_conv(hipStream_t st, const ConvW& c, Loc A, int lda, int M, Loc out, int ldo, int out_C, int epi = EPI_NONE,
                  Loc res = Loc{nullptr, SEG_NONE, 0}, int ldr = 0, const float* scale = nullptr, const Snake* sn = nullptr, bool a_split = false,
                  bool o_split = false) {
        GemmArgs g{};
        g.a_split = a_split ? 1 : 0; g.o_split = o_split ? 1 : 0;
        g.A = A.p; g.lda = lda; g.cin = c.cin; g.dil = c.dil; g.W = c.w.p; g.wscale = c.wsc.p; g.bias = c.b.n ? c.b.p : nullptr; g.out = out.p; g.ldo = ldo;
        g.M = M; g.N = c.N; g.K = c.K; g.epi = epi; g.res = res.p; g.ldr = ldr; g.scale = scale;
        g.a_segT = A.segT; g.a_skip = (int)A.skip_rows;
        g.o_segT = out.segT; g.o_skip = out.skip_rows * out_C;
        g.r_segT = res.segT; g.r_skip = res.skip_rows * ldr;
        if (sn) { g.snake_ea = sn->ea.p; g.snake_ib = sn->inv_eb.p; }
        gemm(st, g, S->splitk_ws.p, S->splitk_ws.n, c.wh.n ? c.wh.p : nullptr, c.wl.n ? c.wl.p : nullptr);
    }
    HistTable table;
    void plan_hist(const Ext& e, int T) {
        if (e.H == 0) return;
        Q3_CHECK(table.n < 48, "too many streaming convolutions");
        Q3_CHECK(e.C % 4 == 0, "streaming state rows must be a multiple of 4 channels (k_hist_all moves float4s)");
        table.d[table.n++] = HistDesc{work(e), e.hist.p, e.H, e.C, T, 0};
    }
    void move_hist(hipStream_t st, int G, const int64_t* meta, bool save) { launch_hist_all(st, table, G, meta, save); }

    void snake(hipStream_t st, const Snake& s, const float* src, float* dst, int rows, RowMap dm, bool split = false) {
        Q3_CHECK(s.C % 4 == 0, "SnakeBeta channel count must be a multiple of 4");
        launch_snake(st, src, dst, s.C, s.ea.p, s.inv_eb.p, rows, dm, split);
    }
    void copy_rows(hipStream_t st, const float* src, float* dst, int rows, int C, RowMap dm) {
        const size_t n = (size_t)rows * C;
        hipLaunchKernelGGL(k_copy_rows, dim3((unsigned)((n + 255) / 256)), dim3(256), 0, st, src, dst, n, C, dm);
    }
};

CodecDecoder::CodecDecoder(const std::string& path, int n_streams, int max_frames, int n_lanes, int max_group) : impl_(new Impl()) {
    Impl& m = *impl_;
    if (const char* e = std::getenv("Q3_CODEC_PRESPLIT")) m.presplit = !(e[0] == '0');
    if (g_codec_f32) m.presplit = false;
    Gguf g(path);
    m.n_streams = n_streams; m.max_frames = max_frames; m.gmax = max_group > 0 ? max_group : 1;
    m.n_q = (int)g.kv_int("codec.n_codebooks", 16); m.cb_size = (int)g.kv_int("codec.codebook_size", 2048);
    m.cb_dim = (int)g.kv_int("codec.codebook_dim", 512); m.hidden = (int)g.kv_int("codec.hidden", 1024);
    m.n_layers = (int)g.kv_int("codec.n_layers", 8); m.n_heads = (int)g.kv_int("codec.n_heads", 16);
    m.head_dim = (int)g.kv_int("codec.head_dim", 64); m.ffn = (int)g.kv_int("codec.ffn", 3072);
    m.window = (int)g.kv_int("codec.window", 72); m.dec_dim = (int)g.kv_int("codec.dec_dim", 1536);
    m.rope_base = (float)g.kv_float("codec.rope_base", 10000.0); m.eps = (float)g.kv_float("codec.eps", 1e-5);
    m.n_up = (int)g.kv_int("codec.n_up", 2); m.n_dec = (int)g.kv_int("codec.n_dec", 4);
    static const int def_rates[8] = {8, 5, 4, 3, 2, 2, 2, 2};
    for (int i = 0; i < m.n_up; i++) m.up_ratios[i] = (int)g.kv_int("codec.up_ratio." + std::to_string(i), 2);
    for (int i = 0; i < m.n_dec; i++) m.dec_rates[i] = (int)g.kv_int("codec.dec_rate." + std::to_string(i), def_rates[i]);
    const int H = m.hidden, A = m.n_heads * m.head_dim;
    Q3_CHECK(A == H && m.head_dim <= 128 && m.window <= 128 && m.cb_dim % 16 == 0 && H % 16 == 0 && m.ffn % 16 == 0, "unsupported codec dims");
    std::vector<const float*> cbp;
    m.codebooks.resize(m.n_q);
    for (int q = 0; q < m.n_q; q++) { Impl::up_f(m.codebooks[q], Impl::tensor(g, "codec.codebook." + std::to_string(q))); cbp.push_back(m.codebooks[q].p); }
    m.d_cb_ptrs.alloc(m.n_q); m.d_cb_ptrs.upload(cbp.data(), m.n_q);
    m.make_conv(m.pre_conv, g, "codec.pre_conv.weight", "codec.pre_conv.bias", H, m.cb_dim, 3, 1);
    m.tf.resize(m.n_layers);
    double fl = 0;
    fl += 2.0 * H * m.cb_dim * 3;
    for (int l = 0; l < m.n_layers; l++) {
        auto& L = m.tf[l];
        const std::string p = "codec.tf." + std::to_string(l) + ".";
        Impl::up_f(L.attn_norm, Impl::tensor(g, p + "attn_norm")); Impl::up_f(L.ffn_norm, Impl::tensor(g, p + "ffn_norm"));
        Impl::up_f(L.ls_attn, Impl::tensor(g, p + "ls_attn")); Impl::up_f(L.ls_ffn, Impl::tensor(g, p + "ls_ffn"));
        auto wq = Impl::tensor(g, p + "wq"), wk = Impl::tensor(g, p + "wk"), wv = Impl::tensor(g, p + "wv");
        std::vector<float> qkv; qkv.insert(qkv.end(), wq.begin(), wq.end()); qkv.insert(qkv.end(), wk.begin(), wk.end()); qkv.insert(qkv.end(), wv.begin(), wv.end());
        m.make_linear(L.wqkv, qkv, 3 * H, H);
        m.make_linear(L.wo, Impl::tensor(g, p + "wo"), H, A);
        auto wg = Impl::tensor(g, p + "w_gate"), wu = Impl::tensor(g, p + "w_up");
        std::vector<float> gu; gu.insert(gu.end(), wg.begin(), wg.end()); gu.insert(gu.end(), wu.begin(), wu.end());
        m.make_linear(L.wgu, gu, 2 * m.ffn, H);
        m.make_linear(L.wdown, Impl::tensor(g, p + "w_down"), H, m.ffn);
        fl += 2.0 * (4.0 * H * H + 3.0 * H * m.ffn);
    }
    Impl::up_f(m.tf_norm, Impl::tensor(g, "codec.tf.norm"));
    {
        std::vector<float> c, s;
        rope_tables(m.head_dim, m.rope_base, Q3TTS_CODEC_MAX_FRAMES, c, s);
        Impl::up_f(m.rope_c, c); Impl::up_f(m.rope_s, s);
    }
    int rate = 1;
    m.up.resize(m.n_up);
    for (int i = 0; i < m.n_up; i++) {
        auto& U = m.up[i];
        const std::string p = "codec.up." + std::to_string(i) + ".";
        const int f = m.up_ratios[i];
        m.make_convt(U.ct, g, p + "convt.weight", p + "convt.bias", H, H, f, f);
        Impl::up_f(U.dw_w, Impl::tensor(g, p + "dw.weight")); Impl::up_f(U.dw_b, Impl::tensor(g, p + "dw.bias"));
        Impl::up_f(U.ln_w, Impl::tensor(g, p + "ln.weight")); Impl::up_f(U.ln_b, Impl::tensor(g, p + "ln.bias"));
        m.make_linear(U.pw1, Impl::tensor(g, p + "pw1.weight"), 4 * H, H); Impl::up_f(U.pw1.b, Impl::tensor(g, p + "pw1.bias"));
        m.make_linear(U.pw2, Impl::tensor(g, p + "pw2.weight"), H, 4 * H); Impl::up_f(U.pw2.b, Impl::tensor(g, p + "pw2.bias"));
        Impl::up_f(U.gamma, Impl::tensor(g, p + "gamma"));
        fl += rate * 2.0 * H * H * f;
        rate *= f;
        fl += rate * 2.0 * (7.0 * H + 8.0 * H * H);
    }
    m.make_conv(m.conv_in, g, "codec.dec.conv_in.weight", "codec.dec.conv_in.bias", m.dec_dim, H, 7, 1);
    fl += rate * 2.0 * 7.0 * H * m.dec_dim;
    int ch = m.dec_dim;
    m.blk.resize(m.n_dec);
    for (int b = 0; b < m.n_dec; b++) {
        auto& B = m.blk[b];
        const std::string p = "codec.dec." + std::to_string(b) + ".";
        const int r = m.dec_rates[b], co = ch / 2;
        B.cin = ch; B.cout = co; B.rate = r;
        m.make_snake(B.snake, g, p + "snake.alpha", p + "snake.beta", ch);
        m.make_convt(B.ct, g, p + "convt.weight", p + "convt.bias", ch, co, 2 * r, r);
        fl += rate * 2.0 * ch * co * 2.0 * r;
        rate *= r;
        static const int dil[3] = {1, 3, 9};
        for (int u = 0; u < 3; u++) {
            const std::string q = p + "ru." + std::to_string(u) + ".";
            m.make_snake(B.ru[u].s1, g, q + "snake1.alpha", q + "snake1.beta", co);
            m.make_conv(B.ru[u].c1, g, q + "conv1.weight", q + "conv1.bias", co, co, 7, dil[u]);
            m.make_snake(B.ru[u].s2, g, q + "snake2.alpha", q + "snake2.beta", co);
            m.make_conv(B.ru[u].c2, g, q + "conv2.weight", q + "conv2.bias", co, co, 1, 1);
            fl += rate * 2.0 * co * co * 8.0;
        }
        ch = co;
    }
    m.make_snake(m.snake_out, g, "codec.dec.snake_out.alpha", "codec.dec.snake_out.beta", ch);
    {
        Q3_CHECK(ch % 4 == 0, "conv_out width must be a multiple of 4 (k_conv_out_wave reads float4 rows)");
        auto w = Impl::tensor(g, "codec.dec.conv_out.weight");
        std::vector<float> r((size_t)7 * ch);
        for (int c = 0; c < ch; c++) for (int j = 0; j < 7; j++) r[(size_t)j * ch + c] = w[(size_t)c * 7 + j];
        Impl::up_f(m.conv_out_w, r);
        m.conv_out_b = Impl::tensor(g, "codec.dec.conv_out.bias")[0];
        fl += rate * 2.0 * 7.0 * ch;
    }
    m.flops_frame = fl;
    const int T0 = max_frames, GM = m.gmax;
    m.make_ext(m.z_ext, 2, m.cb_dim, T0);
    m.k_ext.resize(m.n_layers); m.v_ext.resize(m.n_layers);
    for (int l = 0; l < m.n_layers; l++) { m.make_ext(m.k_ext[l], m.window - 1, H, T0); m.make_ext(m.v_ext[l], m.window - 1, H, T0); }
    int T = T0;
    m.dw_ext.resize(m.n_up);
    for (int i = 0; i < m.n_up; i++) { T *= m.up_ratios[i]; m.make_ext(m.dw_ext[i], 6, H, T); }
    const int Tlat = T;
    m.make_ext(m.convin_ext, 6, H, Tlat);
    m.ct_ext.resize(m.n_dec); m.ru_ext.resize(m.n_dec);
    size_t max_act = (size_t)Tlat * 4 * H;
    ch = m.dec_dim;
    static const int dil[3] = {1, 3, 9};
    for (int b = 0; b < m.n_dec; b++) {
        m.make_ext(m.ct_ext[b], 1, ch, T);
        T *= m.dec_rates[b]; ch /= 2;
        m.ru_ext[b].resize(3);
        for (int u = 0; u < 3; u++) m.make_ext(m.ru_ext[b][u], 6 * dil[u], ch, T);
        max_act = std::max(max_act, (size_t)T * ch);
    }
    m.make_ext(m.out_ext, 6, ch, T);
    max_act = std::max(max_act, (size_t)Tlat * m.dec_dim);
    max_act *= GM;
    m.kv_len.assign(n_streams, 0); m.n_seen.assign(n_streams, 0);
    m.lanes.resize(n_lanes > 0 ? n_lanes : 1);
    for (auto& L : m.lanes) {
        const size_t R0 = (size_t)GM * T0;
        L.h.alloc(R0 * H); L.xn.alloc(R0 * H); L.qkv.alloc(R0 * 3 * H); L.att.alloc(R0 * H);
        L.gu.alloc(R0 * 2 * m.ffn); L.act.alloc(R0 * m.ffn);
        L.t1.alloc(max_act); L.t2.alloc(max_act); L.pcm.alloc((size_t)GM * T);
        L.work.resize(m.all_ext.size());
        for (Ext* e : m.all_ext) L.work[e->id].alloc((size_t)GM * (e->H + e->Tmax) * e->C);
        L.d_in.alloc(m.in_slot());
        L.splitk_ws.alloc(std::max<size_t>(max_act * 2, (size_t)1 << 20));
        Q3_HIP(hipHostMalloc((void**)&L.h_in, (size_t)m.ring * m.in_slot() * sizeof(int64_t)));
    }
    m.S = &m.lanes[0];
    Q3_HIP(hipDeviceSynchronize());
}
CodecDecoder::~CodecDecoder() { if (impl_) for (auto& L : impl_->lanes) if (L.h_in) (void)hipHostFree(L.h_in); }
int CodecDecoder::max_group() const { return impl_->gmax; }
int CodecDecoder::n_lanes() const { return (int)impl_->lanes.size(); }
int CodecDecoder::samples_per_frame() const {
    int s = 1;
    for (int i = 0; i < impl_->n_up; i++) s *= impl_->up_ratios[i];
    for (int i = 0; i < impl_->n_dec; i++) s *= impl_->dec_rates[i];
    return s;
}
double CodecDecoder::flops_per_frame() const { return impl_->flops_frame; }

void CodecDecoder::reset(int s) {
    Impl& m = *impl_;
// ... 79 lines not shown
    flush();
    m.kv_len[s] = 0; m.n_seen[s] = 0;
}

int CodecDecoder::decode(hipStream_t st, int s, const int64_t* codes, int n_frames, bool is_last, float* pcm) {
    const int T = decode_async(st, s, codes, n_frames, is_last, pcm, 0);
    Q3_HIP(hipStreamSynchronize(st));
    return T;
}
int CodecDecoder::decode_async(hipStream_t st, int s, const int64_t* codes, int n_frames, bool is_last, float* pcm, int lane) {
    (void)is_last;
    return decode_group_async(st, 1, &s, codes, n_frames, &pcm, lane);
}

int CodecDecoder::decode_group_async(hipStream_t st, int G, const int* streams, const int64_t* codes, int n_frames, float* const* pcm, int lane) {
    Impl& m = *impl_;
    Q3_CHECK(lane >= 0 && lane < (int)m.lanes.size(), "codec lane out of range");
    Q3_CHECK(G >= 1 && G <= m.gmax, "group size out of range");
    m.S = &m.lanes[lane];
    if (n_frames <= 0) return 0;
    Q3_CHECK(n_frames <= m.max_frames, "too many frames per decode call");
    for (int g = 0; g < G; g++) {
        Q3_CHECK(streams[g] >= 0 && streams[g] < m.n_streams, "stream out of range");
        for (int h = 0; h < g; h++) Q3_CHECK(streams[h] != streams[g], "a stream may appear once per group");
        Q3_CHECK(positions_ok(m.n_seen[streams[g]], n_frames), "codec stream would pass Q3TTS_CODEC_MAX_FRAMES frames (RoPE positions)");
    }
    const int H = m.hidden, T0 = n_frames, R0 = G * T0, W = m.window;
    if (m.S->ring_idx == m.ring) { Q3_HIP(hipStreamSynchronize(st)); m.S->ring_idx = 0; }
    int64_t* hin = m.S->h_in + (size_t)(m.S->ring_idx++) * m.in_slot();
    const size_t ncodes = (size_t)R0 * m.n_q;
    std::copy(codes, codes + ncodes, hin);
    for (int g = 0; g < G; g++) { hin[ncodes + g] = streams[g]; hin[ncodes + G + g] = m.kv_len[streams[g]]; hin[ncodes + 2 * G + g] = m.n_seen[streams[g]]; }
    Q3_HIP(hipMemcpyAsync(m.S->d_in.p, hin, (ncodes + 3 * (size_t)G) * 8, hipMemcpyHostToDevice, st));
    const int64_t* d_codes = m.S->d_in.p;
    const int64_t* meta = m.S->d_in.p + ncodes;
    {
        m.table.n = 0;
        m.plan_hist(m.z_ext, T0);
        for (int l = 0; l < m.n_layers; l++) { m.plan_hist(m.k_ext[l], T0); m.plan_hist(m.v_ext[l], T0); }
        int Tp = T0;
        for (int i = 0; i < m.n_up; i++) { Tp *= m.up_ratios[i]; m.plan_hist(m.dw_ext[i], Tp); }
        m.plan_hist(m.convin_ext, Tp);
        for (int b = 0; b < m.n_dec; b++) {
            m.plan_hist(m.ct_ext[b], Tp);
            Tp *= m.dec_rates[b];
            for (int u = 0; u < 3; u++) m.plan_hist(m.ru_ext[b][u], Tp);
        }
        m.plan_hist(m.out_ext, Tp);
        m.move_hist(st, G, meta, false);
    }
    launch_rvq_sum(st, d_codes, m.d_cb_ptrs.p, m.n_q, m.cb_size, m.cb_dim, R0, m.work(m.z_ext), m.cur_map(m.z_ext, T0));
    m.run_conv(st, m.pre_conv, m.ext_base(m.z_ext, T0), m.cb_dim, R0, m.plain(m.S->h.p), H, H);
    for (int l = 0; l < m.n_layers; l++) {
        auto& L = m.tf[l];
        Ext &ke = m.k_ext[l], &ve = m.v_ext[l];
        launch_rmsnorm(st, m.S->h.p, L.attn_norm.p, H, m.eps, m.S->xn.p, R0);
        m.run_conv(st, L.wqkv, m.plain(m.S->xn.p), H, R0, m.plain(m.S->qkv.p), 3 * H, 3 * H);
        launch_rope_append(st, m.S->qkv.p, H, m.head_dim, m.rope_c.p, m.rope_s.p, meta, G, T0, m.work(ke), m.work(ve), m.cur_map(ke, T0));
        launch_window_attn(st, m.S->qkv.p, m.n_heads, H, m.head_dim, m.work(ke), m.work(ve), meta, G, T0, W, m.S->att.p);
        m.run_conv(st, L.wo, m.plain(m.S->att.p), H, R0, m.plain(m.S->h.p), H, H, EPI_RES_SCALE, m.plain(m.S->h.p), H, L.ls_attn.p);
        launch_rmsnorm(st, m.S->h.p, L.ffn_norm.p, H, m.eps, m.S->xn.p, R0);
        m.run_conv(st, L.wgu, m.plain(m.S->xn.p), H, R0, m.plain(m.S->gu.p), 2 * m.ffn, 2 * m.ffn);
        launch_swiglu(st, m.S->gu.p, m.ffn, m.S->act.p, R0);
        m.run_conv(st, L.wdown, m.plain(m.S->act.p), m.ffn, R0, m.plain(m.S->h.p), H, H, EPI_RES_SCALE, m.plain(m.S->h.p), H, L.ls_ffn.p);
    }
    for (int g = 0; g < G; g++) {
        const int s = streams[g], tot = m.kv_len[s] + T0;
        m.kv_len[s] = tot < W - 1 ? tot : W - 1;
        m.n_seen[s] += T0;
    }
    launch_rmsnorm(st, m.S->h.p, m.tf_norm.p, H, m.eps, m.S->t1.p, R0);
    int T = T0;
    float* x = m.S->t1.p;
    for (int i = 0; i < m.n_up; i++) {
        auto& U = m.up[i];
        const int f = m.up_ratios[i];
        Ext& e = m.dw_ext[i];
        m.run_conv(st, U.ct, m.plain(x), H, G * T, Impl::Loc{m.work(e) + (size_t)e.H * e.C, T, e.H}, f * H, H);
        T *= f;
        launch_dwconv7(st, m.work(e), H, U.dw_w.p, U.dw_b.p, m.S->t2.p, G * T, m.base_map(e, T));
        launch_layernorm(st, m.S->t2.p, U.ln_w.p, U.ln_b.p, H, 1e-6f, m.S->t2.p, G * T);
        float* m1 = m.S->t1.p;
        m.run_conv(st, U.pw1, m.plain(m.S->t2.p), H, G * T, m.plain(m1), 4 * H, 4 * H, EPI_GELU);
        m.run_conv(st, U.pw2, m.plain(m1), 4 * H, G * T, m.plain(m.S->t2.p), H, H, EPI_RES_SCALE, m.ext_cur(e, T), H, U.gamma.p);
        m.copy_rows(st, m.S->t2.p, m.S->t1.p, G * T, H, plain_map());
        x = m.S->t1.p;
    }
    m.copy_rows(st, x, m.work(m.convin_ext), G * T, H, m.cur_map(m.convin_ext, T));
    m.run_conv(st, m.conv_in, m.ext_base(m.convin_ext, T), H, G * T, m.plain(m.S->t1.p), m.dec_dim, m.dec_dim);
    float* d = m.S->t1.p;
    for (int b = 0; b < m.n_dec; b++) {
        auto& B = m.blk[b];
        Ext& ce = m.ct_ext[b];
        m.snake(st, B.snake, d, m.work(ce), G * T, m.cur_map(ce, T), m.presplit);
        float* y = (d == m.S->t1.p) ? m.S->t2.p : m.S->t1.p;
        m.run_conv(st, B.ct, m.ext_base(ce, T), B.cin, G * T, m.plain(y), B.rate * B.cout, B.cout, EPI_NONE, Impl::Loc{nullptr, SEG_NONE, 0}, 0, nullptr, nullptr, m.presplit);
        T *= B.rate;
        for (int u = 0; u < 3; u++) {
            Ext& re = m.ru_ext[b][u];
            auto& R = B.ru[u];
            m.snake(st, R.s1, y, m.work(re), G * T, m.cur_map(re, T), m.presplit);
            float* c1o = d;
            m.run_conv(st, R.c1, m.ext_base(re, T), B.cout, G * T, m.plain(c1o), B.cout, B.cout, EPI_SNAKE, Impl::Loc{nullptr, SEG_NONE, 0}, 0, nullptr, &R.s2, m.presplit, m.presplit);
            m.run_conv(st, R.c2, m.plain(c1o), B.cout, G * T, m.plain(y), B.cout, B.cout, EPI_RES, m.plain(y), B.cout, nullptr, nullptr, m.presplit);
        }
        d = y;
    }
    m.snake(st, m.snake_out, d, m.work(m.out_ext), G * T, m.cur_map(m.out_ext, T));
    launch_conv_out(st, m.work(m.out_ext), m.out_ext.C, m.conv_out_w.p, m.conv_out_b, m.S->pcm.p, G, T, m.base_map(m.out_ext, T), conv_out_win_ok(m.out_ext.C, T));
    m.move_hist(st, G, meta, true);
    Q3_LAUNCH_CHECK();
    for (int g = 0; g < G; g++) Q3_HIP(hipMemcpyAsync(pcm[g], m.S->pcm.p + (size_t)g * T, (size_t)T * 4, hipMemcpyDeviceToHost, st));
    return T;
}

static GemmArgs desc_args(const q3tts_codec_gemm_desc& d) {
    GemmArgs g{};
    g.lda = d.lda; g.cin = d.cin; g.dil = d.dil; g.M = d.M; g.N = d.N; g.K = d.cin * d.taps; g.ldo = d.ldo; g.epi = d.epi; g.ldr = d.ldr;
    g.a_segT = d.a_segT > 0 ? d.a_segT : SEG_NONE; g.a_skip = d.a_segT > 0 ? d.a_skip : 0;
    g.o_segT = d.o_segT > 0 ? d.o_segT : SEG_NONE; g.o_skip = d.o_segT > 0 ? d.o_skip : 0;
    g.r_segT = d.r_segT > 0 ? d.r_segT : SEG_NONE; g.r_skip = d.r_segT > 0 ? d.r_skip : 0;
    g.a_split = d.a_split ? 1 : 0; g.o_split = d.o_split ? 1 : 0;
    g.xcd_swizzle = xcd_swizzle_on();
    return g;
}
static void check_desc(const q3tts_codec_gemm_desc& d) {
    Q3_CHECK(d.M >= 1 && d.N >= 1 && d.cin >= 1 && d.taps >= 1 && d.dil >= 1 && d.epi >= EPI_NONE && d.epi <= EPI_SNAKE, "bad codec GEMM descriptor");
    Q3_CHECK(d.a_segT >= 0 && d.o_segT >= 0 && d.r_segT >= 0 && d.a_skip >= 0 && d.o_skip >= 0 && d.r_skip >= 0 && d.out_off >= 0 && d.ws_floats >= 0,
             "negative segment / offset fields");
    Q3_CHECK(d.A && d.W && d.out && d.lda >= d.cin && d.ldo >= d.N, "codec GEMM: A, W and out are required; lda >= cin, ldo >= N");
    const long long m = d.M - 1;
    const long long arow = m + (d.a_segT > 0 ? m / d.a_segT * d.a_skip : 0) + (long long)(d.taps - 1) * d.dil;
    Q3_CHECK(arow < d.a_rows, "A rows read beyond a_rows");
    Q3_CHECK(d.out_off + m * d.ldo + (d.o_segT > 0 ? m / d.o_segT * d.o_skip : 0) + d.N <= d.out_floats, "output rows beyond out_floats");
    if (d.epi == EPI_RES || d.epi == EPI_RES_SCALE)
        Q3_CHECK(d.res && d.ldr >= d.N && m * d.ldr + (d.r_segT > 0 ? m / d.r_segT * d.r_skip : 0) + d.N <= d.res_floats, "residual rows beyond res_floats");
    Q3_CHECK(d.epi != EPI_RES_SCALE || d.scale, "EPI_RES_SCALE needs scale");
    Q3_CHECK(d.epi != EPI_SNAKE || (d.snake_ea && d.snake_ib), "EPI_SNAKE needs ea / ib");
}
void codec_gemm_plan_only(q3tts_codec_gemm_desc* d) {
    Q3_CHECK(d && d->M >= 1 && d->N >= 1 && d->cin >= 1 && d->taps >= 1 && d->out_off >= 0, "bad codec GEMM descriptor");
    GemmArgs g = desc_args(*d);
    auto at = [](const float* p, long long off) { return reinterpret_cast<float*>((p ? reinterpret_cast<uintptr_t>(p) : (uintptr_t)256) + 4 * (uintptr_t)off); };
    g.A = at(d->A, 0); g.W = at(d->W, 0); g.bias = d->bias; g.res = at(d->res, 0); g.scale = at(d->scale, 0);
    g.snake_ea = at(d->snake_ea, 0); g.snake_ib = at(d->snake_ib, 0); g.out = at(d->out, d->out_off); g.ws = at(nullptr, 0);
    const GemmPlan p = plan_gemm(g, (size_t)d->ws_floats, true);
    d->form_ran = p.form; d->ksplit_ran = p.ks; d->reducer_ran = p.red;
}
void codec_gemm_run(q3tts_codec_gemm_desc* d) {
    Q3_CHECK(d, "null codec GEMM descriptor");
    check_desc(*d);
    GemmArgs g = desc_args(*d);
    const int N = g.N, K = g.K;
    const bool res_used = g.epi == EPI_RES || g.epi == EPI_RES_SCALE;
    DevBuf<float> dA((size_t)d->a_rows * d->lda), dW((size_t)N * K), dsc(N), dbias(d->bias ? N : 0), dres(res_used ? d->res_floats : 0);
    DevBuf<float> dscale(d->scale ? N : 0), dea(d->snake_ea ? N : 0), dib(d->snake_ib ? N : 0), dout(d->out_floats), dws(std::max<int64_t>(d->ws_floats, 4));
    DevBuf<_Float16> dwh((size_t)N * K), dwl((size_t)N * K);
    g.A = dA.p; g.W = dW.p; g.wscale = dsc.p; g.bias = dbias.p; g.res = dres.p; g.scale = dscale.p; g.snake_ea = dea.p; g.snake_ib = dib.p;
    g.out = dout.p + d->out_off; g.ws = dws.p;
    const GemmPlan p = d->form == Q3TTS_GEMM_AUTO ? plan_gemm(g, (size_t)d->ws_floats, true) : GemmPlan{d->form, d->ksplit, d->reducer};
    if (const char* why = gemm_plan_error(g, p, (size_t)d->ws_floats, true)) throw Error(std::string("codec GEMM form not applicable: ") + why);
    std::vector<_Float16> h((size_t)N * K), l((size_t)N * K);
    std::vector<float> sc(N);
    split_weights(d->W, N, K, h.data(), l.data(), sc.data());
    dA.upload(d->A, dA.n); dW.upload(d->W, dW.n); dwh.upload(h.data(), h.size()); dwl.upload(l.data(), l.size()); dsc.upload(sc.data(), N);
    if (d->bias) dbias.upload(d->bias, N);
    if (res_used) dres.upload(d->res, dres.n);
    if (d->scale) dscale.upload(d->scale, N);
    if (d->snake_ea) dea.upload(d->snake_ea, N);
    if (d->snake_ib) dib.upload(d->snake_ib, N);
    dout.upload(d->out, dout.n);
    launch_gemm(0, g, p, dwh.p, dwl.p);
    Q3_LAUNCH_CHECK();
    Q3_HIP(hipDeviceSynchronize());
    dout.download(d->out, dout.n);
    d->form_ran = p.form; d->ksplit_ran = p.ks; d->reducer_ran = p.red;
}

void codec_kernel_run(q3tts_codec_kernel_desc* d) {
    Q3_CHECK(d, "null codec kernel descriptor");
    const int k = d->kernel, G = d->G, T = d->T, C = d->C, H = d->H;
    Q3_CHECK(k >= Q3TTS_CK_RVQ_SUM && k <= Q3TTS_CK_HIST_ZERO, "unknown codec kernel");
    Q3_CHECK(G >= 1 && T >= 1 && C >= 1 && H >= 0 && (long long)G * T <= (1 << 20), "codec kernel: G, T, C >= 1 and H >= 0");
    const long long R = (long long)G * T, ext = (long long)G * (H + T) * C;
    auto need_in = [&](int i, long long n) { Q3_CHECK(d->in[i] && d->in_floats[i] >= n, "codec kernel: in[" + std::to_string(i) + "] missing or too small"); };
    auto need_out = [&](int i, long long n) { Q3_CHECK(d->out[i] && d->out_floats[i] >= n, "codec kernel: out[" + std::to_string(i) + "] missing or too small"); };
    auto need_p = [&](const float* p, int64_t have, long long n) { Q3_CHECK(p && have >= n, "codec kernel: parameter vector missing or too small"); };
    auto need_meta = [&]() { Q3_CHECK(d->meta, "codec kernel: meta is required"); };
    const bool win = k == Q3TTS_CK_CONV_OUT_WIN;
    switch (k) {
    case Q3TTS_CK_RVQ_SUM:
        Q3_CHECK(d->codes && d->n_q >= 1 && d->cb_size >= 1, "RVQ_SUM: codes, n_q and cb_size are required");
        need_in(0, (long long)d->n_q * d->cb_size * C); need_out(0, ext); break;
    case Q3TTS_CK_RMSNORM_ROWS: case Q3TTS_CK_LAYERNORM_ROWS:
        if (d->in[0]) need_in(0, R * C);
        need_p(d->p0, d->p0_floats, C);
        if (k == Q3TTS_CK_LAYERNORM_ROWS) need_p(d->p1, d->p1_floats, C);
        need_out(0, R * C); break;
    case Q3TTS_CK_ROPE_APPEND: case Q3TTS_CK_WINDOW_ATTN:
        Q3_CHECK(d->n_heads >= 1 && d->head_dim >= 2 && d->head_dim % 2 == 0 && (long long)d->n_heads * d->head_dim == C, "C must equal n_heads * head_dim (even)");
        Q3_CHECK(d->window >= 1 && H == d->window - 1, "the K / V extended buffers hold window - 1 history rows");
        need_meta();
        if (k == Q3TTS_CK_ROPE_APPEND) {
            for (int g = 0; g < G; g++)
                Q3_CHECK(positions_ok(d->meta[2 * G + g], T), "ROPE_APPEND: a position reaches Q3TTS_CODEC_MAX_FRAMES (or frames seen < 0)");
            need_out(0, R * 3 * C); need_out(1, ext); need_out(2, ext);
        } else {
            Q3_CHECK(d->head_dim <= 128 && d->window <= 128, "WINDOW_ATTN: head_dim and window must be <= 128 (LDS rows)");
            for (int g = 0; g < G; g++) Q3_CHECK(d->meta[G + g] >= 0 && d->meta[G + g] <= d->window - 1, "WINDOW_ATTN: kv_len outside [0, window)");
            need_in(0, R * 3 * C); need_in(1, ext); need_in(2, ext); need_out(0, R * C);
        }
        break;
    case Q3TTS_CK_SWIGLU_ROWS: need_in(0, R * 2 * C); need_out(0, R * C); break;
    case Q3TTS_CK_DWCONV7:
        Q3_CHECK(H == 6, "DWCONV7: 6 history rows"); need_in(0, ext); need_p(d->p0, d->p0_floats, 7LL * C); need_p(d->p1, d->p1_floats, C); need_out(0, R * C); break;
    case Q3TTS_CK_SNAKE: case Q3TTS_CK_SNAKE_SPLIT:
        Q3_CHECK(C % 4 == 0, "SNAKE: C % 4 == 0 (float4 rows)");
        need_in(0, R * C); need_p(d->p0, d->p0_floats, C); need_p(d->p1, d->p1_floats, C); need_out(0, ext); break;
    case Q3TTS_CK_CONV_OUT_WAVE: case Q3TTS_CK_CONV_OUT_WIN:
        Q3_CHECK(H == 6 && C % 4 == 0, "CONV_OUT: 6 history rows and C % 4 == 0");
        Q3_CHECK(!win || conv_out_win_ok(C, T), "CONV_OUT_WIN: needs C == 96 and T % 128 == 0");
        need_in(0, ext); need_p(d->p0, d->p0_floats, 7LL * C); need_out(0, R); break;
    case Q3TTS_CK_HIST_LOAD: case Q3TTS_CK_HIST_SAVE: case Q3TTS_CK_HIST_ZERO: {
        Q3_CHECK(H >= 1 && C % 4 == 0 && d->n_streams >= 1, "HIST: H >= 1, C % 4 == 0, n_streams >= 1");
        const long long store = (long long)d->n_streams * H * C;
        if (k == Q3TTS_CK_HIST_ZERO) { Q3_CHECK(d->stream >= 0 && d->stream < d->n_streams, "HIST_ZERO: stream out of range"); need_out(0, store); break; }
        need_meta();
        for (int g = 0; g < G; g++) Q3_CHECK(d->meta[g] >= 0 && d->meta[g] < d->n_streams, "HIST: stream slot out of range");
        if (k == Q3TTS_CK_HIST_LOAD) { need_in(0, store); need_out(0, ext); } else { need_in(0, ext); need_out(0, store); }
        break;
    }
    }
    DevBuf<float> din[3], dout[3], dp0, dp1;
    for (int i = 0; i < 3; i++) {
        if (d->in[i] && d->in_floats[i] > 0) { din[i].alloc((size_t)d->in_floats[i]); din[i].upload(d->in[i], din[i].n); }
        if (d->out[i] && d->out_floats[i] > 0) { dout[i].alloc((size_t)d->out_floats[i]); dout[i].upload(d->out[i], dout[i].n); }
    }
    if (d->p0 && d->p0_floats > 0) { dp0.alloc((size_t)d->p0_floats); dp0.upload(d->p0, dp0.n); }
    if (d->p1 && d->p1_floats > 0) { dp1.alloc((size_t)d->p1_floats); dp1.upload(d->p1, dp1.n); }
    DevBuf<int64_t> dmeta, dcodes;
    if (d->meta) { dmeta.alloc(3 * (size_t)G); dmeta.upload(d->meta, dmeta.n); }
    if (k == Q3TTS_CK_RVQ_SUM) { dcodes.alloc((size_t)R * d->n_q); dcodes.upload(d->codes, dcodes.n); }
    const RowMap cur{T, H, H}, base{T, H, 0};
    std::vector<float> rc, rs;
    DevBuf<float> drc, drs;
    DevBuf<const float*> dcb;
    const hipStream_t st = 0;
    switch (k) {
    case Q3TTS_CK_RVQ_SUM: {
        std::vector<const float*> cbp(d->n_q);
        for (int q = 0; q < d->n_q; q++) cbp[q] = din[0].p + (size_t)q * d->cb_size * C;
        dcb.alloc(d->n_q); dcb.upload(cbp.data(), d->n_q);
        launch_rvq_sum(st, dcodes.p, dcb.p, d->n_q, d->cb_size, C, (int)R, dout[0].p, cur);
        break;
    }
    case Q3TTS_CK_RMSNORM_ROWS: launch_rmsnorm(st, d->in[0] ? din[0].p : dout[0].p, dp0.p, C, d->eps, dout[0].p, (int)R); break;
    case Q3TTS_CK_LAYERNORM_ROWS: launch_layernorm(st, d->in[0] ? din[0].p : dout[0].p, dp0.p, dp1.p, C, d->eps, dout[0].p, (int)R); break;
    case Q3TTS_CK_ROPE_APPEND:
        rope_tables(d->head_dim, d->rope_base, Q3TTS_CODEC_MAX_FRAMES, rc, rs);
        drc.alloc(rc.size()); drc.upload(rc.data(), rc.size()); drs.alloc(rs.size()); drs.upload(rs.data(), rs.size());
// ... 23 lines not shown
```

### qwen3-tts-rust_amd/python/q3tts/__init__.py

```python
import ctypes as C
import os
import numpy as np

_HERE = os.path.dirname(os.path.abspath(__file__))
PKG_ROOT = os.path.dirname(os.path.dirname(_HERE))
LIB_PATH = os.path.join(PKG_ROOT, "libq3tts.so")
_lib = None


class Q3Error(RuntimeError):
    pass


class SamplerConfig(C.Structure):
    _fields_ = [("temperature", C.c_float), ("top_k", C.c_int32), ("top_p", C.c_float), ("has_seed", C.c_int32),
                ("seed", C.c_uint64)]


class GenOptions(C.Structure):
    _fields_ = [("repetition_penalty", C.c_float), ("predictor_temperature", C.c_float), ("predictor_top_k", C.c_int32),
                ("predictor_top_p", C.c_float)]


GEN_DEFAULTS = {"repetition_penalty": 1.0, "predictor_temperature": 0.0, "predictor_top_k": 0, "predictor_top_p": 1.0}


class EngineParams(C.Structure):
    _fields_ = [("model_dir", C.c_char_p), ("quant", C.c_char_p), ("device", C.c_int32), ("max_batch", C.c_int32),
                ("max_prompt", C.c_int32), ("max_steps", C.c_int32), ("load_codec", C.c_int32), ("use_graph", C.c_int32)]


class Request(C.Structure):
    _fields_ = [("prompt", C.c_void_p), ("n_prompt", C.c_int32), ("sampler", SamplerConfig), ("max_steps", C.c_int32),
                ("mask_eos", C.c_int32), ("codes_out", C.c_void_p), ("pcm_out", C.c_void_p), ("pcm_capacity", C.c_int64),
                ("n_frames", C.c_int32), ("n_pcm", C.c_int64), ("prefill_ms", C.c_double), ("first_chunk_ms", C.c_double),
                ("total_ms", C.c_double)]


class Stats(C.Structure):
    _fields_ = [("frame_loop_ms", C.c_double), ("frames", C.c_int64), ("prefill_ms", C.c_double), ("gemv_ms", C.c_double),
                ("gemv_launches", C.c_int64), ("gemv_bytes", C.c_double), ("codec_ms", C.c_double), ("codec_calls", C.c_int64),
                ("talker_weight_bytes", C.c_double), ("predictor_weight_bytes", C.c_double), ("kv_bytes_per_token", C.c_double),
                ("gu_ms", C.c_double), ("gu_launches", C.c_int64), ("gu_bytes", C.c_double),
                ("sched_steps", C.c_int64), ("slot_frames", C.c_double), ("graph_frames", C.c_int64)]


class ReqStatus(C.Structure):
    _fields_ = [("state", C.c_int32), ("n_frames", C.c_int32), ("n_pcm", C.c_int64), ("queue_ms", C.c_double),
                ("prefill_ms", C.c_double), ("first_chunk_ms", C.c_double), ("total_ms", C.c_double)]


REQ_QUEUED, REQ_RUNNING, REQ_DRAINING, REQ_DONE, REQ_CANCELLED, REQ_FAILED = 0, 1, 2, 3, 4, -1


DECODE_CB = C.CFUNCTYPE(None, C.c_void_p, C.POINTER(C.c_int64), C.c_int32, C.c_int32)

SYMBOLS = [
    "q3tts_last_error", "q3tts_version", "q3tts_device_count", "q3tts_sampler_config_default", "q3tts_engine_params_default",
    "q3tts_engine_create", "q3tts_engine_destroy", "q3tts_generate_batch", "q3tts_engine_stats", "q3tts_engine_reset_stats",
    "q3tts_engine_set_instrument", "q3tts_engine_bytes_per_step", "q3tts_assets_open", "q3tts_assets_close", "q3tts_engine_assets",
    "q3tts_assets_codec_embedding", "q3tts_assets_text_embedding", "q3tts_assets_tts_pad", "q3tts_prompt_build_core",
    "q3tts_prompt_build_clone", "q3tts_sampler_new", "q3tts_sampler_free", "q3tts_sampler_sample", "q3tts_chunker_new",
    "q3tts_chunker_free", "q3tts_chunker_push", "q3tts_decoder_create", "q3tts_decoder_destroy", "q3tts_decoder_samples_per_frame",
    "q3tts_decoder_reset", "q3tts_decoder_decode", "q3tts_mel_frames", "q3tts_mel", "q3tts_tf_open", "q3tts_tf_close",
    "q3tts_tf_dims", "q3tts_tf_clear", "q3tts_tf_eval", "q3tts_op_gemv_q8", "q3tts_op_gateup_q8", "q3tts_op_matmul_float", "q3tts_op_rmsnorm_quant", "q3tts_op_swiglu_quant",
    "q3tts_op_argmax", "q3tts_op_project", "q3tts_op_sample", "q3tts_submit", "q3tts_poll", "q3tts_fetch", "q3tts_wait",
    "q3tts_release", "q3tts_decoder_create_ex", "q3tts_decoder_decode_group", "q3tts_sched_start", "q3tts_sched_stop", "q3tts_sched_step", "q3tts_voice_register", "q3tts_submit_text",
    "q3tts_group_create", "q3tts_group_destroy", "q3tts_group_size", "q3tts_group_engine", "q3tts_group_uses_rccl", "q3tts_group_voice_register",
    "q3tts_group_submit", "q3tts_group_submit_text", "q3tts_group_device_of", "q3tts_group_poll", "q3tts_group_fetch", "q3tts_group_wait",
    "q3tts_group_release", "q3tts_group_start", "q3tts_group_stop", "q3tts_comm_available", "q3tts_comm_unique_id", "q3tts_comm_create",
    "q3tts_comm_destroy", "q3tts_comm_voice_register", "q3tts_engine_device",
    "q3tts_onnx_open", "q3tts_onnx_close", "q3tts_onnx_counts", "q3tts_onnx_summary", "q3tts_onnx_node", "q3tts_onnx_node_input", "q3tts_onnx_node_output",
    "q3tts_onnx_node_attr_ints", "q3tts_onnx_node_attr_float", "q3tts_onnx_initializer", "q3tts_onnx_op_kernel", "q3tts_onnx_decoder_contract",
    "q3tts_onnx_session_open", "q3tts_onnx_session_close", "q3tts_onnx_session_unsupported", "q3tts_onnx_session_set_input", "q3tts_onnx_session_run",
    "q3tts_onnx_session_output_info", "q3tts_onnx_session_output", "q3tts_onnx_session_launches", "q3tts_onnx_op_executable",
    "q3tts_text_nfc", "q3tts_op_gemv_kq", "q3tts_op_gateup_kq", "q3tts_onnx_decoder_open", "q3tts_onnx_decoder_close", "q3tts_onnx_decoder_reset", "q3tts_onnx_decoder_fetch", "q3tts_group_info", "q3tts_onnx_decoder_decode",
    "q3tts_decoder_state_floats", "q3tts_decoder_state_export", "q3tts_decoder_state_import", "q3tts_decoder_state_entry",
    "q3tts_tokenizer_open", "q3tts_tokenizer_close", "q3tts_tokenizer_encode", "q3tts_tokenizer_decode", "q3tts_tokenizer_vocab_size",
    "q3tts_gen_options_default", "q3tts_submit_ex", "q3tts_submit_text_ex", "q3tts_generate_batch_ex", "q3tts_group_submit_ex",
    "q3tts_group_submit_text_ex", "q3tts_op_sample_rows",
    "q3tts_prompt_build_streaming", "q3tts_submit_trailing", "q3tts_submit_text_streaming", "q3tts_generate_batch_trailing",
    "q3tts_group_submit_text_streaming", "q3tts_op_codec_gemm", "q3tts_codec_gemm_plan", "q3tts_op_codec_kernel", "q3tts_op_attention", "q3tts_attention_plan",
    "q3tts_op_linear", "q3tts_linear_plan", "q3tts_argmax_key",
    "q3tts_submit_trailing_open", "q3tts_trail_append", "q3tts_trail_progress", "q3tts_submit_text_streaming_open", "q3tts_text_append",
    "q3tts_group_submit_text_streaming_open", "q3tts_group_text_append", "q3tts_group_trail_append", "q3tts_group_trail_progress",
    "q3tts_cancel", "q3tts_group_cancel",
    "q3tts_submit_resume", "q3tts_group_submit_resume", "q3tts_op_feedback_rows", "q3tts_engine_prefill_width",
    "q3tts_engine_set_logprobs", "q3tts_fetch_logprobs", "q3tts_group_set_logprobs", "q3tts_group_fetch_logprobs", "q3tts_op_logprob_rows",
    "q3tts_submit_score", "q3tts_group_submit_score", "q3tts_engine_score_width", "q3tts_op_score_rows", "q3tts_op_score_inputs",
    "q3tts_pred_table_bytes", "q3tts_op_attention_keyed", "q3tts_op_select_rows",
    "q3tts_submit_candidates", "q3tts_group_submit_candidates", "q3tts_engine_candidate_stats", "q3tts_op_kv_fork",
    "q3tts_submit_decode", "q3tts_group_submit_decode", "q3tts_engine_decode_width", "q3tts_engine_decode_stats",
]

LOGPROB_COLS = 17
LOGPROB_NONE = 1.0


def lib():
    global _lib
    if _lib is None:
        if not os.path.exists(LIB_PATH):
            raise Q3Error("libq3tts.so not built (run qwen3-tts-rust_amd/build.sh); there is no CPU fallback")
        L = C.CDLL(LIB_PATH)
        L.q3tts_last_error.restype = C.c_char_p
        L.q3tts_engine_create.argtypes = [C.POINTER(EngineParams), C.POINTER(C.c_void_p)]
        L.q3tts_engine_destroy.argtypes = [C.c_void_p]
        L.q3tts_generate_batch.argtypes = [C.c_void_p, C.POINTER(Request), C.c_int32, C.c_int32]
        L.q3tts_engine_stats.argtypes = [C.c_void_p, C.POINTER(Stats)]
        L.q3tts_submit.argtypes = [C.c_void_p, C.POINTER(Request), C.c_int32, C.POINTER(C.c_int64)]
        L.q3tts_poll.argtypes = [C.c_void_p, C.c_int64, C.POINTER(ReqStatus)]
        L.q3tts_fetch.argtypes = [C.c_void_p, C.c_int64, C.c_void_p, C.c_int32, C.c_int32, C.c_void_p, C.c_int64, C.c_int64,
                                  C.POINTER(C.c_int32), C.POINTER(C.c_int64)]
        L.q3tts_wait.argtypes = [C.c_void_p, C.c_int64, C.c_double]
        L.q3tts_release.argtypes = [C.c_void_p, C.c_int64]
        L.q3tts_sched_start.argtypes = [C.c_void_p]
        L.q3tts_sched_stop.argtypes = [C.c_void_p]
        L.q3tts_sched_step.argtypes = [C.c_void_p, C.POINTER(C.c_int32)]
        L.q3tts_voice_register.argtypes = [C.c_void_p, C.c_void_p, C.c_void_p, C.c_int32, C.c_void_p, C.c_int32, C.POINTER(C.c_int32)]
        L.q3tts_submit_text.argtypes = [C.c_void_p, C.c_int32, C.c_void_p, C.c_int32, C.c_int32, C.c_void_p, C.c_int32,
                                        C.POINTER(SamplerConfig), C.c_int32, C.c_int32, C.c_int32, C.POINTER(C.c_int64)]
        L.q3tts_engine_reset_stats.argtypes = [C.c_void_p]
        L.q3tts_engine_set_instrument.argtypes = [C.c_void_p, C.c_int32]
        L.q3tts_engine_bytes_per_step.restype = C.c_double
        L.q3tts_engine_bytes_per_step.argtypes = [C.c_void_p, C.c_int32, C.c_double]
        L.q3tts_assets_open.argtypes = [C.c_char_p, C.POINTER(C.c_void_p)]
        L.q3tts_assets_close.argtypes = [C.c_void_p]
        L.q3tts_engine_assets.restype = C.c_void_p
        L.q3tts_engine_assets.argtypes = [C.c_void_p]
        L.q3tts_assets_codec_embedding.argtypes = [C.c_void_p, C.c_int32, C.c_int32, C.c_void_p]
        L.q3tts_assets_text_embedding.argtypes = [C.c_void_p, C.c_int64, C.c_void_p]
        L.q3tts_assets_tts_pad.argtypes = [C.c_void_p, C.c_void_p]
        L.q3tts_prompt_build_core.argtypes = [C.c_void_p, C.c_void_p, C.c_int32, C.c_int32, C.c_int32, C.c_void_p, C.c_void_p,
                                              C.c_int32, C.c_void_p, C.c_int32, C.c_void_p, C.c_int32]
        L.q3tts_prompt_build_clone.argtypes = [C.c_void_p, C.c_void_p, C.c_int32, C.c_void_p, C.c_int32, C.c_void_p, C.c_int32,
                                               C.c_void_p, C.c_int32, C.c_void_p, C.c_int32, C.c_void_p, C.c_int32]
        L.q3tts_sampler_new.restype = C.c_void_p
        L.q3tts_sampler_new.argtypes = [C.c_float, C.c_int32, C.c_float, C.c_uint64]
        L.q3tts_sampler_free.argtypes = [C.c_void_p]
        L.q3tts_sampler_sample.restype = C.c_int32
        L.q3tts_sampler_sample.argtypes = [C.c_void_p, C.c_void_p, C.c_int32, C.c_int32, C.c_int32]
        L.q3tts_chunker_new.restype = C.c_void_p
        L.q3tts_chunker_new.argtypes = [DECODE_CB, C.c_void_p]
        L.q3tts_chunker_free.argtypes = [C.c_void_p]
        L.q3tts_chunker_push.argtypes = [C.c_void_p, C.c_void_p, C.c_int32, C.c_int32]
        L.q3tts_decoder_create.argtypes = [C.c_char_p, C.c_int32, C.POINTER(C.c_void_p)]
        L.q3tts_decoder_destroy.argtypes = [C.c_void_p]
        L.q3tts_decoder_create_ex.argtypes = [C.c_char_p, C.c_int32, C.c_int32, C.c_int32, C.POINTER(C.c_void_p)]
        L.q3tts_decoder_decode_group.argtypes = [C.c_void_p, C.c_int32, C.c_void_p, C.c_void_p, C.c_int32, C.c_void_p]
        L.q3tts_decoder_samples_per_frame.argtypes = [C.c_void_p]
        L.q3tts_decoder_reset.argtypes = [C.c_void_p, C.c_int32]
        L.q3tts_decoder_decode.argtypes = [C.c_void_p, C.c_int32, C.c_void_p, C.c_int32, C.c_int32, C.c_void_p, C.POINTER(C.c_int64)]
        L.q3tts_mel_frames.argtypes = [C.c_int32]
        L.q3tts_mel.argtypes = [C.c_void_p, C.c_int32, C.c_void_p]
        L.q3tts_tf_open.argtypes = [C.c_char_p, C.c_int32, C.c_int32, C.POINTER(C.c_void_p)]
        L.q3tts_tf_close.argtypes = [C.c_void_p]
        L.q3tts_tf_dims.argtypes = [C.c_void_p] + [C.POINTER(C.c_int32)] * 4
        L.q3tts_tf_clear.argtypes = [C.c_void_p]
        L.q3tts_tf_eval.argtypes = [C.c_void_p, C.c_void_p, C.c_void_p, C.c_int32, C.c_void_p, C.c_void_p, C.c_int32, C.c_int32]
        L.q3tts_op_gemv_q8.argtypes = [C.c_void_p, C.c_int32, C.c_int32, C.c_void_p, C.c_void_p, C.c_int32, C.c_void_p, C.c_int32]
        L.q3tts_op_gateup_q8.argtypes = [C.c_void_p, C.c_int32, C.c_int32, C.c_void_p, C.c_void_p, C.c_int32, C.c_void_p, C.c_void_p]
        L.q3tts_op_matmul_float.argtypes = [C.c_void_p, C.c_int32, C.c_int32, C.c_int32, C.c_int32, C.c_int32, C.c_void_p, C.c_int32, C.c_void_p]
        L.q3tts_op_rmsnorm_quant.argtypes = [C.c_void_p, C.c_void_p, C.c_int32, C.c_int32, C.c_float, C.c_void_p, C.c_void_p, C.c_void_p]
        L.q3tts_op_swiglu_quant.argtypes = [C.c_void_p, C.c_int32, C.c_int32, C.c_void_p, C.c_void_p]
        L.q3tts_op_argmax.argtypes = [C.c_void_p, C.c_int32, C.c_int32, C.c_int32, C.c_int32, C.c_void_p]
        L.q3tts_op_sample.argtypes = [C.c_void_p, C.c_int32, C.c_float, C.c_int32, C.c_float, C.c_uint64, C.c_int32, C.c_int32, C.c_void_p]
        L.q3tts_op_project.argtypes = [C.c_void_p, C.c_void_p, C.c_void_p, C.c_int32, C.c_int32, C.c_void_p]
        L.q3tts_gen_options_default.argtypes = [C.POINTER(GenOptions)]
        L.q3tts_submit_ex.argtypes = [C.c_void_p, C.POINTER(Request), C.c_int32, C.POINTER(GenOptions), C.POINTER(C.c_int64)]
        L.q3tts_submit_text_ex.argtypes = [C.c_void_p, C.c_int32, C.c_void_p, C.c_int32, C.c_int32, C.c_void_p, C.c_int32,
                                           C.POINTER(SamplerConfig), C.c_int32, C.c_int32, C.c_int32, C.POINTER(GenOptions),
                                           C.POINTER(C.c_int64)]
        L.q3tts_generate_batch_ex.argtypes = [C.c_void_p, C.POINTER(Request), C.c_int32, C.c_int32, C.POINTER(GenOptions)]
        L.q3tts_group_submit_ex.argtypes = [C.c_void_p, C.POINTER(Request), C.c_int32, C.POINTER(GenOptions), C.POINTER(C.c_int64)]
        L.q3tts_group_submit_text_ex.argtypes = [C.c_void_p, C.c_int32, C.c_void_p, C.c_int32, C.c_int32, C.c_void_p, C.c_int32,
# ... 712 lines not shown
    p = np.ascontiguousarray(np.broadcast_to(np.asarray(top_p, np.float32), (B,)))
    s = np.ascontiguousarray(np.broadcast_to(np.asarray(seed, np.uint64), (B,)))
    pen = hist = hlen = None
    cap = 1
    if penalty is not None:
        pen = np.ascontiguousarray(np.broadcast_to(np.asarray(penalty, np.float32), (B,)))
        history = history if history is not None else [[] for _ in range(B)]
        cap = max(1, max(len(h) for h in history))
        hist = np.full((B, cap), -1, np.int32)
        hlen = np.array([len(h) for h in history], np.int32)
        for b, h in enumerate(history):
            hist[b, : len(h)] = h
    out = np.zeros((n_draws, B), np.int32)
    _chk(lib().q3tts_op_sample_rows(kernel, _p(lg), B, n, _p(t), _p(k), _p(p), _p(pen), _p(s), _p(hist), _p(hlen), cap, n_draws, _p(out)))
    return out


def op_project(x, w, b):
    x = np.ascontiguousarray(x, np.float32)
    w = np.ascontiguousarray(w, np.float32)
    b = np.ascontiguousarray(b, np.float32)
    y = np.zeros(b.size, np.float32)
    _chk(lib().q3tts_op_project(_p(x), _p(w), _p(b), x.size, b.size, _p(y)))
    return y


GEMM_FORMS = {"AUTO": 0, "SKINNY4": 1, "SKINNY8": 2, "SKINNY16": 3, "F32_1": 4, "F32_2": 5, "H1": 6, "H1_EPL": 7, "H2": 8, "H2_EPL": 9,
              "H3": 10, "H3_EPL": 11}
GEMM_FORM_NAMES = {v: k for k, v in GEMM_FORMS.items()}
EPI_NONE, EPI_GELU, EPI_RES_SCALE, EPI_RES, EPI_SNAKE = range(5)


class CodecGemmDesc(C.Structure):
    _fields_ = [("M", C.c_int32), ("N", C.c_int32), ("cin", C.c_int32), ("taps", C.c_int32), ("dil", C.c_int32),
                ("A", C.c_void_p), ("a_rows", C.c_int64), ("lda", C.c_int32), ("a_segT", C.c_int32), ("a_skip", C.c_int32),
                ("a_split", C.c_int32), ("o_split", C.c_int32),
                ("W", C.c_void_p), ("bias", C.c_void_p),
                ("epi", C.c_int32), ("res", C.c_void_p), ("res_floats", C.c_int64), ("ldr", C.c_int32), ("r_segT", C.c_int32), ("r_skip", C.c_int64),
                ("scale", C.c_void_p), ("snake_ea", C.c_void_p), ("snake_ib", C.c_void_p),
                ("out", C.c_void_p), ("out_floats", C.c_int64), ("out_off", C.c_int64), ("ldo", C.c_int32), ("o_segT", C.c_int32), ("o_skip", C.c_int64),
                ("ws_floats", C.c_int64),
                ("form", C.c_int32), ("ksplit", C.c_int32), ("reducer", C.c_int32),
                ("form_ran", C.c_int32), ("ksplit_ran", C.c_int32), ("reducer_ran", C.c_int32)]


def _codec_gemm_desc(M, N, cin, taps, dil, lda, a_rows, a_segT, a_skip, epi, ldr, res_floats, r_segT, r_skip, ldo, out_floats, out_off,
                     o_segT, o_skip, a_split, o_split, ws_floats, form, ksplit, reducer):
    d = CodecGemmDesc()
    d.M, d.N, d.cin, d.taps, d.dil = M, N, cin, taps, dil
    d.lda, d.a_rows, d.a_segT, d.a_skip = lda, a_rows, a_segT, a_skip
    d.epi, d.ldr, d.res_floats, d.r_segT, d.r_skip = epi, ldr, res_floats, r_segT, r_skip
    d.ldo, d.out_floats, d.out_off, d.o_segT, d.o_skip = ldo, out_floats, out_off, o_segT, o_skip
    d.a_split, d.o_split, d.ws_floats = int(bool(a_split)), int(bool(o_split)), ws_floats
    d.form = GEMM_FORMS[form] if isinstance(form, str) else form
    d.ksplit, d.reducer = ksplit, reducer
    return d


def op_codec_gemm(A, W, M, cin, taps=1, dil=1, out=None, ldo=None, out_off=0, o_segT=0, o_skip=0, a_segT=0, a_skip=0, bias=None,
                  epi=EPI_NONE, res=None, ldr=0, r_segT=0, r_skip=0, scale=None, ea=None, ib=None, a_split=False, o_split=False,
                  ws_floats=1 << 22, form="AUTO", ksplit=1, reducer=-1):
    A = np.ascontiguousarray(A)
    assert A.ndim == 2 and A.dtype.itemsize == 4
    W = np.ascontiguousarray(W, np.float32)
    N = W.shape[0]
    ldo = N if ldo is None else ldo
    if out is None:
        out = np.zeros(out_off + M * ldo, np.float32)
    out = np.array(out, copy=True).reshape(-1)
    assert out.dtype.itemsize == 4
    vecs = [None if v is None else np.ascontiguousarray(v, np.float32) for v in (bias, scale, ea, ib)]
    for v in vecs:
        assert v is None or v.size == N
    res = None if res is None else np.ascontiguousarray(res, np.float32).reshape(-1)
    d = _codec_gemm_desc(M, N, cin, taps, dil, A.shape[1], A.shape[0], a_segT, a_skip, epi, ldr, 0 if res is None else res.size, r_segT, r_skip,
                         ldo, out.size, out_off, o_segT, o_skip, a_split, o_split, ws_floats, form, ksplit, reducer)
    d.A, d.W, d.out, d.res = _p(A), _p(W), _p(out), _p(res)
    d.bias, d.scale, d.snake_ea, d.snake_ib = (_p(v) for v in vecs)
    lib().q3tts_op_codec_gemm.argtypes = [C.POINTER(CodecGemmDesc)]
    _chk(lib().q3tts_op_codec_gemm(C.byref(d)))
    return out, (GEMM_FORM_NAMES[d.form_ran], d.ksplit_ran, d.reducer_ran)


def codec_gemm_plan(M, N, cin, taps=1, dil=1, lda=None, ldo=None, out_off=0, o_segT=0, o_skip=0, a_segT=0, a_skip=0, epi=EPI_NONE, ldr=0,
                    r_segT=0, r_skip=0, a_split=False, o_split=False, ws_floats=1 << 22):
    d = _codec_gemm_desc(M, N, cin, taps, dil, cin if lda is None else lda, 0, a_segT, a_skip, epi, ldr, 0, r_segT, r_skip,
                         N if ldo is None else ldo, 0, out_off, o_segT, o_skip, a_split, o_split, ws_floats, 0, 1, -1)
    lib().q3tts_codec_gemm_plan.argtypes = [C.POINTER(CodecGemmDesc)]
    _chk(lib().q3tts_codec_gemm_plan(C.byref(d)))
    return GEMM_FORM_NAMES[d.form_ran], d.ksplit_ran, d.reducer_ran


CODEC_KERNELS = {"RVQ_SUM": 0, "RMSNORM_ROWS": 1, "LAYERNORM_ROWS": 2, "ROPE_APPEND": 3, "WINDOW_ATTN": 4, "SWIGLU_ROWS": 5, "DWCONV7": 6,
                 "SNAKE": 7, "SNAKE_SPLIT": 8, "CONV_OUT_WAVE": 9, "CONV_OUT_WIN": 10, "HIST_LOAD": 11, "HIST_SAVE": 12, "HIST_ZERO": 13}
CODEC_MAX_FRAMES = 65536


class CodecKernelDesc(C.Structure):
    _fields_ = [("kernel", C.c_int32), ("G", C.c_int32), ("T", C.c_int32), ("C", C.c_int32), ("H", C.c_int32),
                ("n_heads", C.c_int32), ("head_dim", C.c_int32), ("window", C.c_int32), ("rope_base", C.c_float), ("eps", C.c_float),
                ("bias", C.c_float), ("meta", C.c_void_p), ("codes", C.c_void_p), ("n_q", C.c_int32), ("cb_size", C.c_int32),
                ("n_streams", C.c_int32), ("stream", C.c_int32), ("inp", C.c_void_p * 3), ("in_floats", C.c_int64 * 3),
                ("p0", C.c_void_p), ("p1", C.c_void_p), ("p0_floats", C.c_int64), ("p1_floats", C.c_int64),
                ("out", C.c_void_p * 3), ("out_floats", C.c_int64 * 3)]


def op_codec_kernel(kernel, G, T, C_, H=0, ins=(), outs=(), p0=None, p1=None, meta=None, codes=None, n_q=0, cb_size=0, n_heads=0,
                    head_dim=0, window=0, rope_base=10000.0, eps=1e-5, bias=0.0, n_streams=0, stream=0):
    d = CodecKernelDesc()
    d.kernel = CODEC_KERNELS[kernel] if isinstance(kernel, str) else kernel
    d.G, d.T, d.C, d.H = G, T, C_, H
    d.n_heads, d.head_dim, d.window, d.rope_base, d.eps, d.bias = n_heads, head_dim, window, rope_base, eps, bias
    d.n_q, d.cb_size, d.n_streams, d.stream = n_q, cb_size, n_streams, stream
    keep = []
    if meta is not None:
        meta = np.ascontiguousarray(meta, np.int64).reshape(-1)
        assert meta.size == 3 * G
        d.meta = meta.ctypes.data; keep.append(meta)
    if codes is not None:
        codes = np.ascontiguousarray(codes, np.int64).reshape(-1)
        assert codes.size == G * T * n_q
        d.codes = codes.ctypes.data; keep.append(codes)
    for i, a in enumerate(ins):
        if a is not None:
            a = np.ascontiguousarray(a).reshape(-1)
            assert a.dtype.itemsize == 4
            d.inp[i], d.in_floats[i] = a.ctypes.data, a.size; keep.append(a)
    res = []
    for i, a in enumerate(outs):
        a = None if a is None else np.array(a, copy=True).reshape(-1)
        if a is not None:
            assert a.dtype.itemsize == 4
            d.out[i], d.out_floats[i] = a.ctypes.data, a.size
        res.append(a)
    for nm, a in (("p0", p0), ("p1", p1)):
        if a is not None:
            a = np.ascontiguousarray(a, np.float32).reshape(-1)
            setattr(d, nm, a.ctypes.data); setattr(d, nm + "_floats", a.size); keep.append(a)
    lib().q3tts_op_codec_kernel.argtypes = [C.POINTER(CodecKernelDesc)]
    _chk(lib().q3tts_op_codec_kernel(C.byref(d)))
    return res


def mel(audio):
    audio = np.ascontiguousarray(audio, np.float32)
    n = lib().q3tts_mel_frames(audio.size)
    out = np.zeros((n, 128), np.float32)
    _chk(lib().q3tts_mel(_p(audio), audio.size, _p(out)))
    return out


class OnnxSession:

    def __init__(self, path, device=0):
        L = lib()
        L.q3tts_onnx_session_open.argtypes = [C.c_char_p, C.c_int32, C.POINTER(C.c_void_p)]
        L.q3tts_onnx_session_close.argtypes = [C.c_void_p]
        L.q3tts_onnx_session_unsupported.argtypes = [C.c_void_p, C.c_char_p, C.c_int64]
        L.q3tts_onnx_session_set_input.argtypes = [C.c_void_p, C.c_char_p, C.c_int32, C.c_void_p, C.c_void_p, C.c_int32]
        L.q3tts_onnx_session_run.argtypes = [C.c_void_p]
        L.q3tts_onnx_session_output_info.argtypes = [C.c_void_p, C.c_char_p, C.POINTER(C.c_int32), C.POINTER(C.c_int32), C.c_void_p]
        L.q3tts_onnx_session_output.argtypes = [C.c_void_p, C.c_char_p, C.c_void_p, C.c_int64]
        L.q3tts_onnx_session_launches.restype = C.c_int64
        L.q3tts_onnx_session_launches.argtypes = [C.c_void_p]
        h = C.c_void_p()
        _chk(L.q3tts_onnx_session_open(path.encode(), device, C.byref(h)))
# ... 424 lines not shown
```

Measured before the change: 731.0.

## Fold next SnakeBeta activation into codec GEMM epilogue as a second output

Adds an optional second output to the codec GEMM epilogue that applies the following SnakeBeta activation and writes it directly. This lets the codec decoder skip separate snake kernels and their intermediate round trips, and in some places skip the first output entirely. It also batches the float4 epilogue loads (two per thread) so parameter and residual fetches are issued before the math. It is on by default and can be disabled with Q3_CODEC_FOLD; it is turned off when presplit is enabled. The cost is extra epilogue work, more registers and new C API and Python entry points.

```diff
diff --git a/include/q3tts.h b/include/q3tts.h
--- a/include/q3tts.h
+++ b/include/q3tts.h
@@ -342,6 +342,13 @@
 } q3tts_codec_gemm_desc;
 int q3tts_op_codec_gemm(q3tts_codec_gemm_desc* d);
 int q3tts_codec_gemm_plan(q3tts_codec_gemm_desc* d);
+typedef struct q3tts_codec_gemm_desc2 {
+    q3tts_codec_gemm_desc g;
+    float* out2; int64_t out2_floats, out2_off; int32_t ld2, segT2; int64_t skip2;
+    int32_t C2, no_first; const float* ea2; const float* ib2;
+} q3tts_codec_gemm_desc2;
+int q3tts_op_codec_gemm2(q3tts_codec_gemm_desc2* d);
+int q3tts_codec_gemm_plan2(q3tts_codec_gemm_desc2* d);
 
 enum { Q3TTS_CK_RVQ_SUM = 0, Q3TTS_CK_RMSNORM_ROWS = 1, Q3TTS_CK_LAYERNORM_ROWS = 2, Q3TTS_CK_ROPE_APPEND = 3, Q3TTS_CK_WINDOW_ATTN = 4,
        Q3TTS_CK_SWIGLU_ROWS = 5, Q3TTS_CK_DWCONV7 = 6, Q3TTS_CK_SNAKE = 7, Q3TTS_CK_SNAKE_SPLIT = 8, Q3TTS_CK_CONV_OUT_WAVE = 9,
diff --git a/qwen3-tts-rust_amd/csrc/capi_ops.cpp b/qwen3-tts-rust_amd/csrc/capi_ops.cpp
--- a/qwen3-tts-rust_amd/csrc/capi_ops.cpp
+++ b/qwen3-tts-rust_amd/csrc/capi_ops.cpp
@@ -824,6 +824,21 @@
     Q3_API_END(Q3TTS_ERR)
 }
 
+int q3tts_op_codec_gemm2(q3tts_codec_gemm_desc2* d) {
+    Q3_API_BEGIN
+    require_gpu();
+    codec_gemm_run2(d);
+    return Q3TTS_OK;
+    Q3_API_END(Q3TTS_ERR)
+}
+
+int q3tts_codec_gemm_plan2(q3tts_codec_gemm_desc2* d) {
+    Q3_API_BEGIN
+    codec_gemm_plan_only2(d);
+    return Q3TTS_OK;
+    Q3_API_END(Q3TTS_ERR)
+}
+
 int q3tts_op_codec_kernel(q3tts_codec_kernel_desc* d) {
     Q3_API_BEGIN
     require_gpu();
diff --git a/qwen3-tts-rust_amd/csrc/codec.h b/qwen3-tts-rust_amd/csrc/codec.h
--- a/qwen3-tts-rust_amd/csrc/codec.h
+++ b/qwen3-tts-rust_amd/csrc/codec.h
@@ -5,6 +5,7 @@
 #include <vector>
 
 struct q3tts_codec_gemm_desc;
+struct q3tts_codec_gemm_desc2;
 struct q3tts_codec_kernel_desc;
 
 namespace q3 {
@@ -35,6 +36,8 @@
 
 void codec_gemm_run(q3tts_codec_gemm_desc* d);
 void codec_gemm_plan_only(q3tts_codec_gemm_desc* d);
+void codec_gemm_run2(q3tts_codec_gemm_desc2* d);
+void codec_gemm_plan_only2(q3tts_codec_gemm_desc2* d);
 void codec_kernel_run(q3tts_codec_kernel_desc* d);
 
 }
diff --git a/qwen3-tts-rust_amd/csrc/codec.hip b/qwen3-tts-rust_amd/csrc/codec.hip
--- a/qwen3-tts-rust_amd/csrc/codec.hip
+++ b/qwen3-tts-rust_amd/csrc/codec.hip
@@ -25,6 +25,7 @@
     int a_segT, a_skip; int o_segT; long long o_skip; int r_segT; long long r_skip;
     int a_split, o_split;
     int xcd_swizzle;
+    float* out2; int ld2; int segT2; long long skip2; int C2; const float *ea2, *ib2; int no_first;
 };
 #define SEG_NONE 0x3fffffff
 
@@ -42,13 +43,15 @@
     const float2 hi = *reinterpret_cast<const float2*>(base + ci), lo = *reinterpret_cast<const float2*>(base + g.cin + ci);
     return make_float4(hi.x, hi.y, lo.x, lo.y);
 }
-__device__ __forceinline__ void gemm_store(const GemmArgs& g, int row, int col, float v) {
+__device__ __forceinline__ void gemm_store_first(const GemmArgs& g, int row, int col, float v) {
     const size_t o = out_off(g, row, 0);
     if (!g.o_split) { g.out[o + col] = v; return; }
     _Float16* base = reinterpret_cast<_Float16*>(g.out + o);
     const _Float16 hi = (_Float16)v;
     base[col] = hi; base[g.N + col] = (_Float16)(v - (float)hi);
 }
+__device__ __forceinline__ size_t out2_off(const GemmArgs& g, int row) { return (size_t)row * g.ld2 + (size_t)seg_of(row, g.segT2) * g.skip2; }
+__device__ __forceinline__ int snake2_col(const GemmArgs& g, int col) { return g.C2 == g.N ? col : col % g.C2; }
 
 __device__ __forceinline__ float snake_sin(float x) {
     const float n = rintf(x * 0.63661977236758134f);
@@ -61,50 +64,96 @@
     const float v = (q & 1) ? cp : sp;
     return (q & 2) ? -v : v;
 }
+__device__ __forceinline__ float snake_act(float v, float ea, float ib) { const float sn = snake_sin(v * ea); return v + ib * (sn * sn); }
 __device__ __forceinline__ float gemm_epilogue(const GemmArgs& g, float v, int row, int col) {
     if (g.bias) v += g.bias[col];
     if (g.epi == EPI_GELU) v = 0.5f * v * (1.0f + erff(v * 0.70710678118654752f));
     else if (g.epi == EPI_RES_SCALE) v = g.res[(size_t)row * g.ldr + (size_t)seg_of(row, g.r_segT) * g.r_skip + col] + g.scale[col] * v;
     else if (g.epi == EPI_RES) v = g.res[(size_t)row * g.ldr + (size_t)seg_of(row, g.r_segT) * g.r_skip + col] + v;
-    else if (g.epi == EPI_SNAKE) { const float sn = snake_sin(v * g.snake_ea[col]); v = v + g.snake_ib[col] * (sn * sn); }
+    else if (g.epi == EPI_SNAKE) v = snake_act(v, g.snake_ea[col], g.snake_ib[col]);
     return v;
 }
 
+__device__ __forceinline__ void gemm_store(const GemmArgs& g, int row, int col, float v) {
+    if (!g.no_first) gemm_store_first(g, row, col, v);
+    if (g.out2) { const int c2 = snake2_col(g, col); g.out2[out2_off(g, row) + col] = snake_act(v, g.ea2[c2], g.ib2[c2]); }
+}
+
 typedef _Float16 h4e_ __attribute__((ext_vector_type(4)));
+struct Epi4 { float4 bias, res, p0, p1, ea2, ib2; };
+__device__ __forceinline__ Epi4 epilogue4_load(const GemmArgs& g, int row, int col) {
+    Epi4 L;
+    const float4 z = make_float4(0.f, 0.f, 0.f, 0.f);
+    L.bias = z; L.res = z; L.p0 = z; L.p1 = z; L.ea2 = z; L.ib2 = z;
+    if (g.bias) L.bias = *reinterpret_cast<const float4*>(g.bias + col);
+    if (g.epi == EPI_RES_SCALE || g.epi == EPI_RES) {
+        L.res = *reinterpret_cast<const float4*>(g.res + (size_t)row * g.ldr + (size_t)seg_of(row, g.r_segT) * g.r_skip + col);
+        if (g.epi == EPI_RES_SCALE) L.p0 = *reinterpret_cast<const float4*>(g.scale + col);
+    } else if (g.epi == EPI_SNAKE) { L.p0 = *reinterpret_cast<const float4*>(g.snake_ea + col); L.p1 = *reinterpret_cast<const float4*>(g.snake_ib + col); }
+    if (g.out2) {
+        const int c2 = snake2_col(g, col);
+        L.ea2 = *reinterpret_cast<const float4*>(g.ea2 + c2); L.ib2 = *reinterpret_cast<const float4*>(g.ib2 + c2);
+    }
+    return L;
+}
+__device__ __forceinline__ void epilogue4_finish(const GemmArgs& g, float4 t, const Epi4& L, int row, int col) {
+    float v[4] = {t.x, t.y, t.z, t.w};
+    if (g.bias) { v[0] += L.bias.x; v[1] += L.bias.y; v[2] += L.bias.z; v[3] += L.bias.w; }
+    if (g.epi == EPI_GELU) {
+#pragma unroll
+        for (int c = 0; c < 4; c++) v[c] = 0.5f * v[c] * (1.0f + erff(v[c] * 0.70710678118654752f));
+    } else if (g.epi == EPI_RES_SCALE) {
+        v[0] = L.res.x + L.p0.x * v[0]; v[1] = L.res.y + L.p0.y * v[1]; v[2] = L.res.z + L.p0.z * v[2]; v[3] = L.res.w + L.p0.w * v[3];
+    } else if (g.epi == EPI_RES) { v[0] = L.res.x + v[0]; v[1] = L.res.y + v[1]; v[2] = L.res.z + v[2]; v[3] = L.res.w + v[3]; }
+    else if (g.epi == EPI_SNAKE) {
+        const float eav[4] = {L.p0.x, L.p0.y, L.p0.z, L.p0.w}, ibv[4] = {L.p1.x, L.p1.y, L.p1.z, L.p1.w};
+#pragma unroll
+        for (int c = 0; c < 4; c++) v[c] = snake_act(v[c], eav[c], ibv[c]);
+    }
+    if (!g.no_first) {
+        const size_t o = out_off(g, row, 0);
+        if (!g.o_split) *reinterpret_cast<float4*>(g.out + o + col) = make_float4(v[0], v[1], v[2], v[3]);
+        else {
+            _Float16* base = reinterpret_cast<_Float16*>(g.out + o);
+            h4e_ hi, lo;
+#pragma unroll
+            for (int c = 0; c < 4; c++) { hi[c] = (_Float16)v[c]; lo[c] = (_Float16)(v[c] - (float)hi[c]); }
+            *reinterpret_cast<h4e_*>(base + col) = hi;
+            *reinterpret_cast<h4e_*>(base + g.N + col) = lo;
+        }
+    }
+    if (g.out2)
+        *reinterpret_cast<float4*>(g.out2 + out2_off(g, row) + col) =
+            make_float4(snake_act(v[0], L.ea2.x, L.ib2.x), snake_act(v[1], L.ea2.y, L.ib2.y), snake_act(v[2], L.ea2.z, L.ib2.z), snake_act(v[3], L.ea2.w, L.ib2.w));
+}
 __device__ __forceinline__ void gemm_epilogue_store4(const GemmArgs& g, float4 t, int row, int col) {
-    float v[4] = {t.x, t.y, t.z, t.w};
-    if (g.bias) { const float4 b = *reinterpret_cast<const float4*>(g.bias + col); v[0] += b.x; v[1] += b.y; v[2] += b.z; v[3] += b.w; }
-    if (g.epi == EPI_GELU) {
-#pragma unroll
-        for (int c = 0; c < 4; c++) v[c] = 0.5f * v[c] * (1.0f + erff(v[c] * 0.70710678118654752f));
-    } else if (g.epi == EPI_RES_SCALE || g.epi == EPI_RES) {
-        const float4 rs = *reinterpret_cast<const float4*>(g.res + (size_t)row * g.ldr + (size_t)seg_of(row, g.r_segT) * g.r_skip + col);
-        if (g.epi == EPI_RES_SCALE) {
-            const float4 sc = *reinterpret_cast<const float4*>(g.scale + col);
-            v[0] = rs.x + sc.x * v[0]; v[1] = rs.y + sc.y * v[1]; v[2] = rs.z + sc.z * v[2]; v[3] = rs.w + sc.w * v[3];
-        } else { v[0] = rs.x + v[0]; v[1] = rs.y + v[1]; v[2] = rs.z + v[2]; v[3] = rs.w + v[3]; }
-    } else if (g.epi == EPI_SNAKE) {
-        const float4 ea = *reinterpret_cast<const float4*>(g.snake_ea + col), ib = *reinterpret_cast<const float4*>(g.snake_ib + col);
-        const float eav[4] = {ea.x, ea.y, ea.z, ea.w}, ibv[4] = {ib.x, ib.y, ib.z, ib.w};
-#pragma unroll
-        for (int c = 0; c < 4; c++) { const float sn = snake_sin(v[c] * eav[c]); v[c] = v[c] + ibv[c] * (sn * sn); }
-    }
-    const size_t o = out_off(g, row, 0);
-    if (!g.o_split) *reinterpret_cast<float4*>(g.out + o + col) = make_float4(v[0], v[1], v[2], v[3]);
-    else {
-        _Float16* base = reinterpret_cast<_Float16*>(g.out + o);
-        h4e_ hi, lo;
-#pragma unroll
-        for (int c = 0; c < 4; c++) { hi[c] = (_Float16)v[c]; lo[c] = (_Float16)(v[c] - (float)hi[c]); }
-        *reinterpret_cast<h4e_*>(base + col) = hi;
-        *reinterpret_cast<h4e_*>(base + g.N + col) = lo;
+    epilogue4_finish(g, t, epilogue4_load(g, row, col), row, col);
+}
+constexpr int EPI_U = 2;
+template <int BM, int BN, int CLD>
+__device__ __forceinline__ void store4_batch(const GemmArgs& g, const float (*Ct)[CLD], int m0, int n0, int tid) {
+    constexpr int C4 = BN / 4;
+    static_assert((BM * C4) % (256 * EPI_U) == 0, "whole batches");
+    for (int e0 = tid; e0 < BM * C4; e0 += 256 * EPI_U) {
+        Epi4 L[EPI_U];
+#pragma unroll
+        for (int u = 0; u < EPI_U; u++) {
+            const int e = e0 + 256 * u, row = m0 + e / C4, col = n0 + (e % C4) * 4;
+            L[u] = epilogue4_load(g, row < g.M ? row : g.M - 1, col < g.N ? col : 0);
+        }
+#pragma unroll
+        for (int u = 0; u < EPI_U; u++) {
+            const int e = e0 + 256 * u, rl = e / C4, cl = (e % C4) * 4, row = m0 + rl, col = n0 + cl;
+            if (row < g.M && col < g.N) epilogue4_finish(g, *reinterpret_cast<const float4*>(&Ct[rl][cl]), L[u], row, col);
+        }
     }
 }
 static bool epilogue4_ok(const GemmArgs& g) {
     auto a16 = [](const void* p) { return (reinterpret_cast<uintptr_t>(p) & 15) == 0; };
     return g.N % 4 == 0 && g.ldo % 4 == 0 && g.o_skip % 4 == 0 && a16(g.out) && (!g.bias || a16(g.bias)) &&
            (!(g.epi == EPI_RES || g.epi == EPI_RES_SCALE) || (g.ldr % 4 == 0 && g.r_skip % 4 == 0 && a16(g.res))) &&
-           (g.epi != EPI_RES_SCALE || a16(g.scale)) && (g.epi != EPI_SNAKE || (a16(g.snake_ea) && a16(g.snake_ib)));
+           (g.epi != EPI_RES_SCALE || a16(g.scale)) && (g.epi != EPI_SNAKE || (a16(g.snake_ea) && a16(g.snake_ib))) &&
+           (!g.out2 || (g.ld2 % 4 == 0 && g.skip2 % 4 == 0 && g.C2 % 4 == 0 && a16(g.out2) && a16(g.ea2) && a16(g.ib2)));
 }
 
 template <int WM>
@@ -473,12 +522,11 @@
             for (int r = 0; r < 16; r++) Ct[wave * 32 + (r & 3) + 8 * (r >> 2) + 4 * (lane >> 5)][u * 32 + (lane & 31)] = acc[0][u][r];
         __syncthreads();
         constexpr int C4 = BN / 4;
-        for (int e = tid; e < BM * C4; e += 256) {
+        if (ksplit == 1) store4_batch<BM, BN, BN + 4>(g, Ct, m0, n0, tid);
+        else for (int e = tid; e < BM * C4; e += 256) {
             const int rl = e / C4, col = n0 + (e % C4) * 4, row = m0 + rl;
             if (row >= g.M) continue;
-            const float4 t4 = *reinterpret_cast<const float4*>(&Ct[rl][(e % C4) * 4]);
-            if (ksplit > 1) *reinterpret_cast<float4*>(g.ws + ((size_t)blockIdx.z * g.M + row) * g.N + col) = t4;
-            else gemm_epilogue_store4(g, t4, row, col);
+            *reinterpret_cast<float4*>(g.ws + ((size_t)blockIdx.z * g.M + row) * g.N + col) = *reinterpret_cast<const float4*>(&Ct[rl][(e % C4) * 4]);
         }
     } else {
         epilogue_rows(acc[0], m0 + wave * MR * 32);
@@ -603,6 +651,9 @@
     if (g.M < 1 || g.N < 1 || g.cin < 4 || g.K % g.cin != 0 || g.dil < 1) return "bad GEMM shape";
     if (g.cin % 4 != 0 || g.lda % 4 != 0 || g.lda < g.cin) return "A rows need cin % 4 == 0 and lda % 4 == 0, lda >= cin";
     if (p.ks < 1 || g.K % p.ks != 0) return "ksplit must divide K";
+    if (g.out2 && (!g.ea2 || !g.ib2 || g.C2 < 4 || g.C2 % 4 != 0 || g.N % g.C2 != 0 || g.ld2 < g.N))
+        return "second output: needs ea2 / ib2, C2 % 4 == 0, N a multiple of C2 and ld2 >= N";
+    if (g.no_first && !g.out2) return "no_first without a second output";
     const bool skinny = f <= Q3TTS_GEMM_SKINNY16, f32 = f == Q3TTS_GEMM_F32_1 || f == Q3TTS_GEMM_F32_2, h3 = f >= Q3TTS_GEMM_H3;
     const bool epl = f == Q3TTS_GEMM_H1_EPL || f == Q3TTS_GEMM_H2_EPL || f == Q3TTS_GEMM_H3_EPL;
     const bool ws_a16 = (reinterpret_cast<uintptr_t>(g.ws) & 15) == 0;
@@ -797,8 +848,7 @@
     const int c4 = C >> 2, c = (int)(i % c4) * 4, r = (int)(i / c4);
     const float4 v = reinterpret_cast<const float4*>(src)[i];
     const float4 a = *reinterpret_cast<const float4*>(ea + c), b = *reinterpret_cast<const float4*>(inv_eb + c);
-    const float s0 = snake_sin(v.x * a.x), s1 = snake_sin(v.y * a.y), s2 = snake_sin(v.z * a.z), s3 = snake_sin(v.w * a.w);
-    const float4 y = make_float4(v.x + b.x * (s0 * s0), v.y + b.y * (s1 * s1), v.z + b.z * (s2 * s2), v.w + b.w * (s3 * s3));
+    const float4 y = make_float4(snake_act(v.x, a.x, b.x), snake_act(v.y, a.y, b.y), snake_act(v.z, a.z, b.z), snake_act(v.w, a.w, b.w));
     float* drow = dst + map_row(dm, r) * C;
     if (!split) { *reinterpret_cast<float4*>(drow + c) = y; return; }
     _Float16* row = reinterpret_cast<_Float16*>(drow);
@@ -961,6 +1011,7 @@
     Snake snake_out; DevBuf<float> conv_out_w; float conv_out_b = 0;
     Ext z_ext, convin_ext, out_ext; std::vector<Ext> dw_ext, ct_ext, k_ext, v_ext; std::vector<std::vector<Ext>> ru_ext;
     std::vector<Ext*> all_ext;
+    bool fold = true;
     bool presplit = false;
     std::vector<int> kv_len; std::vector<long long> n_seen;
     int gmax = 1;
@@ -1036,10 +1087,16 @@
     Loc ext_cur(const Ext& e, int T) { return Loc{work(e) + (size_t)e.H * e.C, T, e.H}; }
     RowMap cur_map(const Ext& e, int T) { return RowMap{T, e.H, e.H}; }
     RowMap base_map(const Ext& e, int T) { return RowMap{T, e.H, 0}; }
+    struct Next { const Snake* sn; Loc out; bool only; };
     void run_conv(hipStream_t st, const ConvW& c, Loc A, int lda, int M, Loc out, int ldo, int out_C, int epi = EPI_NONE,
                   Loc res = Loc{nullptr, SEG_NONE, 0}, int ldr = 0, const float* scale = nullptr, const Snake* sn = nullptr, bool a_split = false,
-                  bool o_split = false) {
+                  bool o_split = false, Next next = Next{nullptr, Loc{nullptr, SEG_NONE, 0}, false}) {
         GemmArgs g{};
+        if (next.sn) {
+            Q3_CHECK(next.sn->C % 4 == 0 && c.N % next.sn->C == 0, "folded SnakeBeta: channel count must be a multiple of 4 and divide N");
+            g.out2 = next.out.p; g.ld2 = c.N; g.segT2 = next.out.segT; g.skip2 = next.out.skip_rows * next.sn->C; g.C2 = next.sn->C;
+            g.ea2 = next.sn->ea.p; g.ib2 = next.sn->inv_eb.p; g.no_first = next.only ? 1 : 0;
+        }
         g.a_split = a_split ? 1 : 0; g.o_split = o_split ? 1 : 0;
         g.A = A.p; g.lda = lda; g.cin = c.cin; g.dil = c.dil; g.W = c.w.p; g.wscale = c.wsc.p; g.bias = c.b.n ? c.b.p : nullptr; g.out = out.p; g.ldo = ldo;
         g.M = M; g.N = c.N; g.K = c.K; g.epi = epi; g.res = res.p; g.ldr = ldr; g.scale = scale;
@@ -1072,6 +1129,8 @@
     Impl& m = *impl_;
     if (const char* e = std::getenv("Q3_CODEC_PRESPLIT")) m.presplit = !(e[0] == '0');
     if (g_codec_f32) m.presplit = false;
+    if (const char* e = std::getenv("Q3_CODEC_FOLD")) m.fold = !(e[0] == '0');
+    if (m.presplit) m.fold = false;
     Gguf g(path);
     m.n_streams = n_streams; m.max_frames = max_frames; m.gmax = max_group > 0 ? max_group : 1;
     m.n_q = (int)g.kv_int("codec.n_codebooks", 16); m.cb_size = (int)g.kv_int("codec.codebook_size", 2048);
@@ -1135,6 +1194,7 @@
     fl += rate * 2.0 * 7.0 * H * m.dec_dim;
     int ch = m.dec_dim;
     m.blk.resize(m.n_dec);
+    if (m.n_dec < 1) m.fold = false;
     for (int b = 0; b < m.n_dec; b++) {
         auto& B = m.blk[b];
         const std::string p = "codec.dec." + std::to_string(b) + ".";
@@ -1380,31 +1440,46 @@
         launch_layernorm(st, m.S->t2.p, U.ln_w.p, U.ln_b.p, H, 1e-6f, m.S->t2.p, G * T);
         float* m1 = m.S->t1.p;
         m.run_conv(st, U.pw1, m.plain(m.S->t2.p), H, G * T, m.plain(m1), 4 * H, 4 * H, EPI_GELU);
+        if (m.fold) {
+            if (i + 1 == m.n_up) m.run_conv(st, U.pw2, m.plain(m1), 4 * H, G * T, m.ext_cur(m.convin_ext, T), H, H, EPI_RES_SCALE, m.ext_cur(e, T), H, U.gamma.p);
+            else m.run_conv(st, U.pw2, m.plain(m1), 4 * H, G * T, m.plain(m.S->t2.p), H, H, EPI_RES_SCALE, m.ext_cur(e, T), H, U.gamma.p);
+            x = m.S->t2.p;
+            continue;
+        }
         m.run_conv(st, U.pw2, m.plain(m1), 4 * H, G * T, m.plain(m.S->t2.p), H, H, EPI_RES_SCALE, m.ext_cur(e, T), H, U.gamma.p);
         m.copy_rows(st, m.S->t2.p, m.S->t1.p, G * T, H, plain_map());
         x = m.S->t1.p;
     }
-    m.copy_rows(st, x, m.work(m.convin_ext), G * T, H, m.cur_map(m.convin_ext, T));
-    m.run_conv(st, m.conv_in, m.ext_base(m.convin_ext, T), H, G * T, m.plain(m.S->t1.p), m.dec_dim, m.dec_dim);
+    const Impl::Loc none{nullptr, SEG_NONE, 0};
+    if (!m.fold || m.n_up == 0) m.copy_rows(st, x, m.work(m.convin_ext), G * T, H, m.cur_map(m.convin_ext, T));
+    if (m.fold) m.run_conv(st, m.conv_in, m.ext_base(m.convin_ext, T), H, G * T, m.plain(m.S->t1.p), m.dec_dim, m.dec_dim, EPI_NONE, none, 0, nullptr, nullptr, false, false,
+                           Impl::Next{&m.blk[0].snake, m.ext_cur(m.ct_ext[0], T), true});
+    else m.run_conv(st, m.conv_in, m.ext_base(m.convin_ext, T), H, G * T, m.plain(m.S->t1.p), m.dec_dim, m.dec_dim);
     float* d = m.S->t1.p;
     for (int b = 0; b < m.n_dec; b++) {
         auto& B = m.blk[b];
         Ext& ce = m.ct_ext[b];
-        m.snake(st, B.snake, d, m.work(ce), G * T, m.cur_map(ce, T), m.presplit);
+        if (!m.fold) m.snake(st, B.snake, d, m.work(ce), G * T, m.cur_map(ce, T), m.presplit);
         float* y = (d == m.S->t1.p) ? m.S->t2.p : m.S->t1.p;
-        m.run_conv(st, B.ct, m.ext_base(ce, T), B.cin, G * T, m.plain(y), B.rate * B.cout, B.cout, EPI_NONE, Impl::Loc{nullptr, SEG_NONE, 0}, 0, nullptr, nullptr, m.presplit);
+        const Impl::Next ct_next = m.fold ? Impl::Next{&B.ru[0].s1, Impl::Loc{m.work(m.ru_ext[b][0]) + (size_t)m.ru_ext[b][0].H * B.cout, T, m.ru_ext[b][0].H}, false}
+                                          : Impl::Next{nullptr, none, false};
+        m.run_conv(st, B.ct, m.ext_base(ce, T), B.cin, G * T, m.plain(y), B.rate * B.cout, B.cout, EPI_NONE, none, 0, nullptr, nullptr, m.presplit, false, ct_next);
         T *= B.rate;
         for (int u = 0; u < 3; u++) {
             Ext& re = m.ru_ext[b][u];
             auto& R = B.ru[u];
-            m.snake(st, R.s1, y, m.work(re), G * T, m.cur_map(re, T), m.presplit);
+            if (!m.fold) m.snake(st, R.s1, y, m.work(re), G * T, m.cur_map(re, T), m.presplit);
             float* c1o = d;
-            m.run_conv(st, R.c1, m.ext_base(re, T), B.cout, G * T, m.plain(c1o), B.cout, B.cout, EPI_SNAKE, Impl::Loc{nullptr, SEG_NONE, 0}, 0, nullptr, &R.s2, m.presplit, m.presplit);
-            m.run_conv(st, R.c2, m.plain(c1o), B.cout, G * T, m.plain(y), B.cout, B.cout, EPI_RES, m.plain(y), B.cout, nullptr, nullptr, m.presplit);
+            m.run_conv(st, R.c1, m.ext_base(re, T), B.cout, G * T, m.plain(c1o), B.cout, B.cout, EPI_SNAKE, none, 0, nullptr, &R.s2, m.presplit, m.presplit);
+            Impl::Next nx{nullptr, none, false};
+            if (m.fold) nx = u < 2 ? Impl::Next{&B.ru[u + 1].s1, m.ext_cur(m.ru_ext[b][u + 1], T), false}
+                           : b + 1 < m.n_dec ? Impl::Next{&m.blk[b + 1].snake, m.ext_cur(m.ct_ext[b + 1], T), true}
+                                             : Impl::Next{&m.snake_out, m.ext_cur(m.out_ext, T), true};
+            m.run_conv(st, R.c2, m.plain(c1o), B.cout, G * T, m.plain(y), B.cout, B.cout, EPI_RES, m.plain(y), B.cout, nullptr, nullptr, m.presplit, false, nx);
         }
         d = y;
     }
-    m.snake(st, m.snake_out, d, m.work(m.out_ext), G * T, m.cur_map(m.out_ext, T));
+    if (!m.fold) m.snake(st, m.snake_out, d, m.work(m.out_ext), G * T, m.cur_map(m.out_ext, T));
     launch_conv_out(st, m.work(m.out_ext), m.out_ext.C, m.conv_out_w.p, m.conv_out_b, m.S->pcm.p, G, T, m.base_map(m.out_ext, T), conv_out_win_ok(m.out_ext.C, T));
     m.move_hist(st, G, meta, true);
     Q3_LAUNCH_CHECK();
@@ -1412,7 +1487,7 @@
     return T;
 }
 
-static GemmArgs desc_args(const q3tts_codec_gemm_desc& d) {
+static GemmArgs desc_args(const q3tts_codec_gemm_desc& d, const q3tts_codec_gemm_desc2* x = nullptr) {
     GemmArgs g{};
     g.lda = d.lda; g.cin = d.cin; g.dil = d.dil; g.M = d.M; g.N = d.N; g.K = d.cin * d.taps; g.ldo = d.ldo; g.epi = d.epi; g.ldr = d.ldr;
     g.a_segT = d.a_segT > 0 ? d.a_segT : SEG_NONE; g.a_skip = d.a_segT > 0 ? d.a_skip : 0;
@@ -1420,6 +1495,9 @@
     g.r_segT = d.r_segT > 0 ? d.r_segT : SEG_NONE; g.r_skip = d.r_segT > 0 ? d.r_skip : 0;
     g.a_split = d.a_split ? 1 : 0; g.o_split = d.o_split ? 1 : 0;
     g.xcd_swizzle = xcd_swizzle_on();
+    if (x) {
+        g.ld2 = x->ld2; g.segT2 = x->segT2 > 0 ? x->segT2 : SEG_NONE; g.skip2 = x->segT2 > 0 ? x->skip2 : 0; g.C2 = x->C2; g.no_first = x->no_first ? 1 : 0;
+    }
     return g;
 }
 static void check_desc(const q3tts_codec_gemm_desc& d) {
@@ -1436,19 +1514,30 @@
     Q3_CHECK(d.epi != EPI_RES_SCALE || d.scale, "EPI_RES_SCALE needs scale");
     Q3_CHECK(d.epi != EPI_SNAKE || (d.snake_ea && d.snake_ib), "EPI_SNAKE needs ea / ib");
 }
-void codec_gemm_plan_only(q3tts_codec_gemm_desc* d) {
+static void check_desc2(const q3tts_codec_gemm_desc2& x) {
+    const q3tts_codec_gemm_desc& d = x.g;
+    Q3_CHECK(x.out2 && x.ea2 && x.ib2, "codec GEMM: the second output needs out2, ea2 and ib2");
+    Q3_CHECK(x.segT2 >= 0 && x.skip2 >= 0 && x.out2_off >= 0 && x.C2 >= 1 && x.ld2 >= d.N, "second output: negative segment / offset fields, C2 < 1 or ld2 < N");
+    const long long m = d.M - 1;
+    Q3_CHECK(x.out2_off + m * x.ld2 + (x.segT2 > 0 ? m / x.segT2 * x.skip2 : 0) + d.N <= x.out2_floats, "second output rows beyond out2_floats");
+}
+static void plan_only(q3tts_codec_gemm_desc* d, const q3tts_codec_gemm_desc2* x) {
     Q3_CHECK(d && d->M >= 1 && d->N >= 1 && d->cin >= 1 && d->taps >= 1 && d->out_off >= 0, "bad codec GEMM descriptor");
-    GemmArgs g = desc_args(*d);
+    GemmArgs g = desc_args(*d, x);
     auto at = [](const float* p, long long off) { return reinterpret_cast<float*>((p ? reinterpret_cast<uintptr_t>(p) : (uintptr_t)256) + 4 * (uintptr_t)off); };
     g.A = at(d->A, 0); g.W = at(d->W, 0); g.bias = d->bias; g.res = at(d->res, 0); g.scale = at(d->scale, 0);
     g.snake_ea = at(d->snake_ea, 0); g.snake_ib = at(d->snake_ib, 0); g.out = at(d->out, d->out_off); g.ws = at(nullptr, 0);
+    if (x) { Q3_CHECK(x->out2_off >= 0, "bad codec GEMM descriptor"); g.out2 = at(x->out2, x->out2_off); g.ea2 = at(x->ea2, 0); g.ib2 = at(x->ib2, 0); }
     const GemmPlan p = plan_gemm(g, (size_t)d->ws_floats, true);
     d->form_ran = p.form; d->ksplit_ran = p.ks; d->reducer_ran = p.red;
 }
-void codec_gemm_run(q3tts_codec_gemm_desc* d) {
+void codec_gemm_plan_only(q3tts_codec_gemm_desc* d) { plan_only(d, nullptr); }
+void codec_gemm_plan_only2(q3tts_codec_gemm_desc2* x) { Q3_CHECK(x, "null codec GEMM descriptor"); plan_only(&x->g, x); }
+static void gemm_run(q3tts_codec_gemm_desc* d, q3tts_codec_gemm_desc2* x) {
     Q3_CHECK(d, "null codec GEMM descriptor");
     check_desc(*d);
-    GemmArgs g = desc_args(*d);
+    if (x) check_desc2(*x);
+    GemmArgs g = desc_args(*d, x);
     const int N = g.N, K = g.K;
     const bool res_used = g.epi == EPI_RES || g.epi == EPI_RES_SCALE;
     DevBuf<float> dA((size_t)d->a_rows * d->lda), dW((size_t)N * K), dsc(N), dbias(d->bias ? N : 0), dres(res_used ? d->res_floats : 0);
@@ -1456,6 +1545,8 @@
     DevBuf<_Float16> dwh((size_t)N * K), dwl((size_t)N * K);
     g.A = dA.p; g.W = dW.p; g.wscale = dsc.p; g.bias = dbias.p; g.res = dres.p; g.scale = dscale.p; g.snake_ea = dea.p; g.snake_ib = dib.p;
     g.out = dout.p + d->out_off; g.ws = dws.p;
+    DevBuf<float> dout2(x ? x->out2_floats : 0), dea2(x ? x->C2 : 0), dib2(x ? x->C2 : 0);
+    if (x) { g.out2 = dout2.p + x->out2_off; g.ea2 = dea2.p; g.ib2 = dib2.p; }
     const GemmPlan p = d->form == Q3TTS_GEMM_AUTO ? plan_gemm(g, (size_t)d->ws_floats, true) : GemmPlan{d->form, d->ksplit, d->reducer};
     if (const char* why = gemm_plan_error(g, p, (size_t)d->ws_floats, true)) throw Error(std::string("codec GEMM form not applicable: ") + why);
     std::vector<_Float16> h((size_t)N * K), l((size_t)N * K);
@@ -1468,12 +1559,16 @@
     if (d->snake_ea) dea.upload(d->snake_ea, N);
     if (d->snake_ib) dib.upload(d->snake_ib, N);
     dout.upload(d->out, dout.n);
+    if (x) { dout2.upload(x->out2, dout2.n); dea2.upload(x->ea2, x->C2); dib2.upload(x->ib2, x->C2); }
     launch_gemm(0, g, p, dwh.p, dwl.p);
     Q3_LAUNCH_CHECK();
     Q3_HIP(hipDeviceSynchronize());
     dout.download(d->out, dout.n);
+    if (x) dout2.download(x->out2, dout2.n);
     d->form_ran = p.form; d->ksplit_ran = p.ks; d->reducer_ran = p.red;
 }
+void codec_gemm_run(q3tts_codec_gemm_desc* d) { gemm_run(d, nullptr); }
+void codec_gemm_run2(q3tts_codec_gemm_desc2* x) { Q3_CHECK(x, "null codec GEMM descriptor"); gemm_run(&x->g, x); }
 
 void codec_kernel_run(q3tts_codec_kernel_desc* d) {
     Q3_CHECK(d, "null codec kernel descriptor");
diff --git a/qwen3-tts-rust_amd/python/q3tts/__init__.py b/qwen3-tts-rust_amd/python/q3tts/__init__.py
--- a/qwen3-tts-rust_amd/python/q3tts/__init__.py
+++ b/qwen3-tts-rust_amd/python/q3tts/__init__.py
@@ -91,6 +91,7 @@
     "q3tts_pred_table_bytes", "q3tts_op_attention_keyed", "q3tts_op_select_rows",
     "q3tts_submit_candidates", "q3tts_group_submit_candidates", "q3tts_engine_candidate_stats", "q3tts_op_kv_fork",
     "q3tts_submit_decode", "q3tts_group_submit_decode", "q3tts_engine_decode_width", "q3tts_engine_decode_stats",
+    "q3tts_op_codec_gemm2", "q3tts_codec_gemm_plan2",
 ]
 
 LOGPROB_COLS = 17
@@ -969,6 +970,53 @@
     return out, (GEMM_FORM_NAMES[d.form_ran], d.ksplit_ran, d.reducer_ran)
 
 
+class CodecGemmDesc2(C.Structure):
+    _fields_ = [("g", CodecGemmDesc), ("out2", C.c_void_p), ("out2_floats", C.c_int64), ("out2_off", C.c_int64), ("ld2", C.c_int32),
+                ("segT2", C.c_int32), ("skip2", C.c_int64), ("C2", C.c_int32), ("no_first", C.c_int32), ("ea2", C.c_void_p), ("ib2", C.c_void_p)]
+
+
+def op_codec_gemm2(A, W, M, cin, out2, ea2, ib2, ld2, out2_off=0, segT2=0, skip2=0, no_first=False, taps=1, dil=1, out=None, ldo=None,
+                   out_off=0, o_segT=0, o_skip=0, a_segT=0, a_skip=0, bias=None, epi=EPI_NONE, res=None, ldr=0, r_segT=0, r_skip=0, scale=None,
+                   ea=None, ib=None, a_split=False, o_split=False, ws_floats=1 << 22, form="AUTO", ksplit=1, reducer=-1):
+    A = np.ascontiguousarray(A)
+    assert A.ndim == 2 and A.dtype.itemsize == 4
+    W = np.ascontiguousarray(W, np.float32)
+    N = W.shape[0]
+    ldo = N if ldo is None else ldo
+    if out is None:
+        out = np.zeros(out_off + M * ldo, np.float32)
+    out = np.array(out, copy=True).reshape(-1)
+    out2 = np.array(out2, copy=True).reshape(-1)
+    assert out.dtype.itemsize == 4 and out2.dtype.itemsize == 4
+    vecs = [None if v is None else np.ascontiguousarray(v, np.float32) for v in (bias, scale, ea, ib)]
+    for v in vecs:
+        assert v is None or v.size == N
+    ea2, ib2 = np.ascontiguousarray(ea2, np.float32), np.ascontiguousarray(ib2, np.float32)
+    assert ea2.size == ib2.size
+    res = None if res is None else np.ascontiguousarray(res, np.float32).reshape(-1)
+    d = CodecGemmDesc2()
+    d.g = _codec_gemm_desc(M, N, cin, taps, dil, A.shape[1], A.shape[0], a_segT, a_skip, epi, ldr, 0 if res is None else res.size, r_segT,
+                           r_skip, ldo, out.size, out_off, o_segT, o_skip, a_split, o_split, ws_floats, form, ksplit, reducer)
+    d.g.A, d.g.W, d.g.out, d.g.res = _p(A), _p(W), _p(out), _p(res)
+    d.g.bias, d.g.scale, d.g.snake_ea, d.g.snake_ib = (_p(v) for v in vecs)
+    d.out2, d.out2_floats, d.out2_off, d.ld2, d.segT2, d.skip2 = _p(out2), out2.size, out2_off, ld2, segT2, skip2
+    d.C2, d.no_first, d.ea2, d.ib2 = ea2.size, int(bool(no_first)), _p(ea2), _p(ib2)
+    lib().q3tts_op_codec_gemm2.argtypes = [C.POINTER(CodecGemmDesc2)]
+    _chk(lib().q3tts_op_codec_gemm2(C.byref(d)))
+    return out, out2, (GEMM_FORM_NAMES[d.g.form_ran], d.g.ksplit_ran, d.g.reducer_ran)
+
+
+def codec_gemm_plan2(M, N, cin, C2, ld2=None, out2_off=0, segT2=0, skip2=0, no_first=False, taps=1, dil=1, lda=None, ldo=None, out_off=0,
+                     o_segT=0, o_skip=0, a_segT=0, a_skip=0, epi=EPI_NONE, ldr=0, r_segT=0, r_skip=0, ws_floats=1 << 22):
+    d = CodecGemmDesc2()
+    d.g = _codec_gemm_desc(M, N, cin, taps, dil, cin if lda is None else lda, 0, a_segT, a_skip, epi, ldr, 0, r_segT, r_skip,
+                           N if ldo is None else ldo, 0, out_off, o_segT, o_skip, False, False, ws_floats, 0, 1, -1)
+    d.out2_off, d.ld2, d.segT2, d.skip2, d.C2, d.no_first = out2_off, N if ld2 is None else ld2, segT2, skip2, C2, int(bool(no_first))
+    lib().q3tts_codec_gemm_plan2.argtypes = [C.POINTER(CodecGemmDesc2)]
+    _chk(lib().q3tts_codec_gemm_plan2(C.byref(d)))
+    return GEMM_FORM_NAMES[d.g.form_ran], d.g.ksplit_ran, d.g.reducer_ran
+
+
 def codec_gemm_plan(M, N, cin, taps=1, dil=1, lda=None, ldo=None, out_off=0, o_segT=0, o_skip=0, a_segT=0, a_skip=0, epi=EPI_NONE, ldr=0,
                     r_segT=0, r_skip=0, a_split=False, o_split=False, ws_floats=1 << 22):
     d = _codec_gemm_desc(M, N, cin, taps, dil, cin if lda is None else lda, 0, a_segT, a_skip, epi, ldr, 0, r_segT, r_skip,
```

Result: no change. 733.2 (median of 3 runs) (+0.3%).
